# automl/TransformersCanDoBayesianInference

Hardware: NVIDIA H100
Metric: prior-sampled sequences/sec, full training step (prior sample + fwd + bwd + allreduce + clip + Adam) (higher is better)
Workload: dtype bf16

## Files before the change

### transformerscandobayesianinference_b200/csrc/attention_bwd_tc.cu

```cuda
#include "attention_common.cuh"

namespace pfn {

constexpr int AB_ROWS = 64;
constexpr int AB_TILE = AB_ROWS * ATT_ROW_BYTES;
constexpr int AB_THREADS = 3 * 128;
constexpr int AB_DQ_STAGES = 4;
constexpr int AB_DKV_STAGES = 3;
constexpr int AB_DQ_OFF_RING = 4 * AB_TILE;
constexpr int AB_DQ_OFF_BAR = AB_DQ_OFF_RING + AB_DQ_STAGES * 2 * AB_TILE;
constexpr int AB_DQ_SMEM = AB_DQ_OFF_BAR + (2 * AB_DQ_STAGES + 2) * 8 + 1024;
constexpr int AB_DKV_OFF_RING = 4 * AB_TILE;
constexpr int AB_DKV_OFF_STAT = AB_DKV_OFF_RING + AB_DKV_STAGES * 2 * AB_TILE;
constexpr int AB_DKV_OFF_BAR = AB_DKV_OFF_STAT + AB_DKV_STAGES * 2 * AB_ROWS * 4;
constexpr int AB_DKV_SMEM = AB_DKV_OFF_BAR + (2 * AB_DKV_STAGES + 1) * 8 + 1024;
static_assert(AB_DQ_SMEM <= 232448 && AB_DKV_SMEM <= 232448, "the tiles and rings must fit the 227 KB of shared memory");

struct AttnBwdParams {
  int T, B, H, sep;
  float scale, scale_log2;
  const __nv_bfloat16* qkv; int ld_qkv;
  const __nv_bfloat16* dout; int ld_dout;
  __nv_bfloat16* dqkv; int ld_dqkv;
  const float* lse;
  const float* delta;
  int delta_tm;
  float* dq_colsum;
  uint32_t drop_seed; int drop_thr;
  int n_tiles;
  int batch_major;
};

__device__ __forceinline__ float ab_delta(const AttnBwdParams& p, int b, int h, int i) {
  return p.delta_tm ? p.delta[att_tok(i, b, p.T, p.B, 0) * p.H + h] : p.delta[(static_cast<size_t>(b) * p.H + h) * p.T + i];
}

__device__ __forceinline__ uint64_t ab_desc_k(uint32_t tile, int kk) {
  return tc::wgmma_smem_desc(tile + (kk >> 2) * 8192 + (kk & 3) * 32, 16, 1024);
}
__device__ __forceinline__ uint64_t ab_desc_mn(uint32_t tile, int kk) {
  return tc::wgmma_smem_desc(tile + kk * 2048, 8192, 1024);
}
__device__ __forceinline__ uint32_t ab_opaque(uint32_t addr) {
  asm volatile("" : "+r"(addr));
  return addr;
}
__device__ __forceinline__ void ab_mma_n64(float (&d)[32], uint64_t a_desc, uint64_t b_desc, int kk) {
  if (kk == 0) tc::wgmma_m64n64k16<0>(d, a_desc, b_desc);
  else tc::wgmma_m64n64k16<1>(d, a_desc, b_desc);
}

__device__ __forceinline__ void ab_load_tile(uint8_t* dst, const CUtensorMap* m, uint64_t* bar, int col0, int b, int t0) {
  tc::tma_load_3d(dst, m, bar, col0, b, t0);
  tc::tma_load_3d(dst + 8192, m, bar, col0 + 64, b, t0);
}

__global__ void __launch_bounds__(256)
attn_bwd_delta_kernel(const __nv_bfloat16* __restrict__ out, int ld_out, const __nv_bfloat16* __restrict__ dout,
                      int ld_dout, float* __restrict__ delta, int T, int B, int H, int batch_major) {
  const int lane = threadIdx.x & 31;
  const long long warp = (static_cast<long long>(blockIdx.x) * blockDim.x + threadIdx.x) >> 5;
  const long long nwarps = (static_cast<long long>(gridDim.x) * blockDim.x) >> 5;
  const long long rows = static_cast<long long>(T) * B;
  for (long long tok = warp; tok < rows; tok += nwarps) {
    const int t = batch_major ? static_cast<int>(tok % T) : static_cast<int>(tok / B);
    const int b = batch_major ? static_cast<int>(tok / T) : static_cast<int>(tok % B);
    for (int h0 = 0; h0 < H; h0 += 2) {
      const int h = h0 + (lane >> 4);
      float acc = 0.f;
      if (h < H) {
        const int col = h * ATT_DH + (lane & 15) * 8;
        const uint4 pa = *reinterpret_cast<const uint4*>(out + tok * ld_out + col);
        const uint4 pb = *reinterpret_cast<const uint4*>(dout + tok * ld_dout + col);
        const __nv_bfloat162* ha = reinterpret_cast<const __nv_bfloat162*>(&pa);
        const __nv_bfloat162* hb = reinterpret_cast<const __nv_bfloat162*>(&pb);
#pragma unroll
        for (int j = 0; j < 4; ++j) {
          const float2 x = __bfloat1622float2(ha[j]);
          const float2 y = __bfloat1622float2(hb[j]);
          acc = fmaf(x.x, y.x, acc);
          acc = fmaf(x.y, y.y, acc);
        }
      }
#pragma unroll
      for (int o = 8; o > 0; o >>= 1) acc += __shfl_xor_sync(0xffffffffu, acc, o);
      if ((lane & 15) == 0 && h < H) delta[(static_cast<size_t>(b) * H + h) * T + t] = acc;
    }
  }
}

__global__ void __launch_bounds__(AB_THREADS, 1)
attn_bwd_dq_kernel(const __grid_constant__ CUtensorMap tmQ, const __grid_constant__ CUtensorMap tmKV,
                   const __grid_constant__ CUtensorMap tmDO, const AttnBwdParams p) {
  extern __shared__ uint8_t smem_raw[];
  uint8_t* smem = smem_raw + ((1024u - (tc::smem_u32(smem_raw) & 1023u)) & 1023u);
  uint8_t* sQ = smem;
  uint8_t* sD = smem + 2 * AB_TILE;
  uint8_t* sRing = smem + AB_DQ_OFF_RING;
  uint64_t* kv_full = reinterpret_cast<uint64_t*>(smem + AB_DQ_OFF_BAR);
  uint64_t* kv_empty = kv_full + AB_DQ_STAGES;
  uint64_t* q_full = kv_empty + AB_DQ_STAGES;
  uint64_t* q_empty = q_full + 1;
  const int warp = threadIdx.x >> 5, lane = threadIdx.x & 31;
  const int E = p.H * ATT_DH;
  const int nblk = (p.sep + AB_ROWS - 1) / AB_ROWS;
  const int n_units = p.n_tiles * p.B * p.H;
  if (threadIdx.x == 0) {
    for (int s = 0; s < AB_DQ_STAGES; ++s) {
      tc::mbar_init(&kv_full[s], 1);
      tc::mbar_init(&kv_empty[s], 2);
    }
    tc::mbar_init(q_full, 1);
    tc::mbar_init(q_empty, 2);
    tc::mbar_fence_init();
  }
  __syncthreads();

  if (warp >= 8) {
    tc::setmaxnreg_dec<40>();
    if (threadIdx.x == 256) {
      tc::tma_prefetch_desc(&tmQ);
      tc::tma_prefetch_desc(&tmKV);
      tc::tma_prefetch_desc(&tmDO);
      int stage = 0;
      uint32_t phase = 0;
      for (int u = blockIdx.x, it = 0; u < n_units; u += gridDim.x, ++it) {
        const int qt = u % p.n_tiles, bh = u / p.n_tiles;
        const int h = bh % p.H, b = bh / p.H;
        auto load_q = [&]() {
          if (it > 0) tc::mbar_wait_suspend(q_empty, (it - 1) & 1);
          tc::mbar_expect_tx(q_full, 4 * AB_TILE);
          for (int g = 0; g < 2; ++g) {
            ab_load_tile(sQ + g * AB_TILE, &tmQ, q_full, h * ATT_DH, b, qt * 128 + 64 * g);
            ab_load_tile(sD + g * AB_TILE, &tmDO, q_full, h * ATT_DH, b, qt * 128 + 64 * g);
          }
        };
        const int claim_at = min(AB_DQ_STAGES - 1, nblk - 1);
        if (nblk == 0) load_q();
        for (int kb = 0; kb < nblk; ++kb) {
          if (kb == claim_at) load_q();
          tc::mbar_wait_suspend(&kv_empty[stage], phase ^ 1);
          uint8_t* dst = sRing + stage * 2 * AB_TILE;
          tc::mbar_expect_tx(&kv_full[stage], 2 * AB_TILE);
          ab_load_tile(dst, &tmKV, &kv_full[stage], E + h * ATT_DH, b, kb * AB_ROWS);
          ab_load_tile(dst + AB_TILE, &tmKV, &kv_full[stage], 2 * E + h * ATT_DH, b, kb * AB_ROWS);
          if (++stage == AB_DQ_STAGES) { stage = 0; phase ^= 1; }
        }
      }
    }
    return;
  }

  tc::setmaxnreg_inc<232>();
  const int g = warp >> 2, wq = warp & 3;
  const int tid = threadIdx.x & 127;
  const uint32_t q_tile = tc::smem_u32(sQ + g * AB_TILE), d_tile = tc::smem_u32(sD + g * AB_TILE);
  const float dscale = p.drop_thr > 0 ? drop_scale(p.drop_thr) : 1.0f;
  int stage = 0;
  uint32_t phase = 0;
  bool timed_out = false;
  for (int u = blockIdx.x, it = 0; u < n_units && !timed_out; u += gridDim.x, ++it) {
    const int qt = u % p.n_tiles, bh = u / p.n_tiles;
    const int h = bh % p.H, b = bh / p.H;
    const int i0 = qt * 128 + 64 * g + 16 * wq + (lane >> 2);

    float lse2[2], dl[2];
    uint32_t drow[2];
#pragma unroll
    for (int r = 0; r < 2; ++r) {
      const int i = i0 + 8 * r;
      const bool valid = i < p.T;
      lse2[r] = valid ? p.lse[static_cast<size_t>(bh) * p.T + i] * 1.4426950408889634f : INFINITY;
      dl[r] = valid ? ab_delta(p, b, h, i) : 0.f;
      drow[r] = static_cast<uint32_t>(bh) * p.T + i;
    }
    if (!tc::mbar_wait_bounded(q_full, it & 1)) { timed_out = true; break; }

    float dq[64];
    for (int kb = 0; kb < nblk; ++kb) {
      if (!tc::mbar_wait_bounded(&kv_full[stage], phase)) { timed_out = true; break; }
      const uint32_t k_s = tc::smem_u32(sRing + stage * 2 * AB_TILE);
      const uint32_t v_s = k_s + AB_TILE;
      const uint32_t q_s = ab_opaque(q_tile), d_s = ab_opaque(d_tile);
      float s[32], dp[32];
      tc::wgmma_fence();
#pragma unroll
      for (int kk = 0; kk < 8; ++kk) ab_mma_n64(s, ab_desc_k(q_s, kk), ab_desc_k(k_s, kk), kk);
#pragma unroll
      for (int kk = 0; kk < 8; ++kk) ab_mma_n64(dp, ab_desc_k(d_s, kk), ab_desc_k(v_s, kk), kk);
      tc::wgmma_commit();
      tc::wgmma_wait<0>();
      tc::wgmma_fence_regs(s);
      tc::wgmma_fence_regs(dp);
      if (kb == nblk - 1 && tid == 0) tc::mbar_arrive(q_empty);

      uint32_t ads[16];
      const int key0 = kb * AB_ROWS + 2 * (lane & 3);
#pragma unroll
      for (int j = 0; j < 8; ++j)
#pragma unroll
        for (int e = 0; e < 4; e += 2) {
          float v[2];
#pragma unroll
          for (int c = 0; c < 2; ++c) {
            const int key = key0 + 8 * j + c;
            const float pr = key < p.sep ? fast_ex2(fmaf(s[4 * j + e + c], p.scale_log2, -lse2[e >> 1])) : 0.f;
            const float mk = p.drop_thr > 0 ? (drop_keep(p.drop_seed, drow[e >> 1], key, p.drop_thr) ? dscale : 0.f) : 1.f;
            v[c] = pr * fmaf(mk, dp[4 * j + e + c], -dl[e >> 1]) * p.scale;
          }
          ads[2 * j + (e >> 1)] = tc::pack_bf16x2(v[0], v[1]);
        }
      tc::wgmma_fence();
#pragma unroll
      for (int kk = 0; kk < 4; ++kk) tc::wgmma_m64n128k16_rs(dq, ads + 4 * kk, ab_desc_mn(k_s, kk), kb > 0 || kk > 0);
      tc::wgmma_commit();
      tc::wgmma_wait<0>();
      if (tid == 0) tc::mbar_arrive(&kv_empty[stage]);
      if (++stage == AB_DQ_STAGES) { stage = 0; phase ^= 1; }
    }
    tc::wgmma_fence_regs(dq);
    if (nblk == 0 && tid == 0) tc::mbar_arrive(q_empty);

    float cs[16][2];
#pragma unroll
    for (int j = 0; j < 16; ++j) cs[j][0] = cs[j][1] = 0.f;
#pragma unroll
    for (int r = 0; r < 2; ++r) {
      const int i = i0 + 8 * r;
      const bool valid = i < p.T;
      const bool diag = valid && i >= p.sep;
      const size_t tok = att_tok(valid ? i : 0, b, p.T, p.B, p.batch_major);
      const __nv_bfloat16* qrow = p.qkv + tok * p.ld_qkv + h * ATT_DH;
      const __nv_bfloat16* drw = p.dout + tok * p.ld_dout + h * ATT_DH;
      __nv_bfloat16* grow = p.dqkv + tok * p.ld_dqkv + h * ATT_DH;
      float sd = 0.f, dpd = 0.f;
      if (diag) {
#pragma unroll
        for (int j = 0; j < 16; ++j) {
          const float2 q = att_ld2(qrow, j, lane), k = att_ld2(qrow + E, j, lane);
          const float2 gr = att_ld2(drw, j, lane), v = att_ld2(qrow + 2 * E, j, lane);
          sd = fmaf(q.x, k.x, fmaf(q.y, k.y, sd));
          dpd = fmaf(gr.x, v.x, fmaf(gr.y, v.y, dpd));
        }
      }
      sd = quad_sum(sd);
      dpd = quad_sum(dpd);
      float ds = 0.f;
      if (diag) {
        const float pr = fast_ex2(fmaf(sd, p.scale_log2, -lse2[r]));
        const float mk = p.drop_thr > 0 ? (drop_keep(p.drop_seed, drow[r], i, p.drop_thr) ? dscale : 0.f) : 1.f;
        ds = pr * fmaf(mk, dpd, -dl[r]) * p.scale;
        const float pm = pr * mk;
#pragma unroll
        for (int j = 0; j < 16; ++j) {
          const float2 q = att_ld2(qrow, j, lane), gr = att_ld2(drw, j, lane);
          att_st2(grow + E, j, lane, ds * q.x, ds * q.y);
          att_st2(grow + 2 * E, j, lane, pm * gr.x, pm * gr.y);
        }
      }
      if (valid) {
#pragma unroll
        for (int j = 0; j < 16; ++j) {
          float x = nblk > 0 ? dq[4 * j + 2 * r] : 0.f, y = nblk > 0 ? dq[4 * j + 2 * r + 1] : 0.f;
          if (diag) {
            const float2 k = att_ld2(qrow + E, j, lane);
            x = fmaf(ds, k.x, x);
            y = fmaf(ds, k.y, y);
          }
          att_st2(grow, j, lane, x, y);
          cs[j][0] += __bfloat162float(__float2bfloat16_rn(x));
          cs[j][1] += __bfloat162float(__float2bfloat16_rn(y));
        }
      }
    }
    if (p.dq_colsum != nullptr) {
#pragma unroll
      for (int j = 0; j < 16; ++j)
#pragma unroll
        for (int e = 0; e < 2; ++e) {
          float v = cs[j][e];
          v += __shfl_xor_sync(0xffffffffu, v, 4);
          v += __shfl_xor_sync(0xffffffffu, v, 8);
          v += __shfl_xor_sync(0xffffffffu, v, 16);
          if (lane < 4) atomicAdd(p.dq_colsum + h * ATT_DH + 8 * j + 2 * lane + e, v);
        }
    }
  }
  if (timed_out) asm volatile("trap;");
}

__global__ void __launch_bounds__(AB_THREADS, 1)
attn_bwd_dkv_kernel(const __grid_constant__ CUtensorMap tmQ, const __grid_constant__ CUtensorMap tmKV,
                    const __grid_constant__ CUtensorMap tmDO, const AttnBwdParams p) {
  extern __shared__ uint8_t smem_raw[];
  uint8_t* smem = smem_raw + ((1024u - (tc::smem_u32(smem_raw) & 1023u)) & 1023u);
  uint8_t* sK = smem;
  uint8_t* sV = smem + 2 * AB_TILE;
  uint8_t* sRing = smem + AB_DKV_OFF_RING;
  float* sStat = reinterpret_cast<float*>(smem + AB_DKV_OFF_STAT);
  uint64_t* full = reinterpret_cast<uint64_t*>(smem + AB_DKV_OFF_BAR);
  uint64_t* empty = full + AB_DKV_STAGES;
  uint64_t* kv_bar = empty + AB_DKV_STAGES;
  const int warp = threadIdx.x >> 5, lane = threadIdx.x & 31;
  const int kt = static_cast<int>(blockIdx.x) % p.n_tiles;
  const int bh = static_cast<int>(blockIdx.x) / p.n_tiles;
  const int h = bh % p.H, b = bh / p.H;
  const int E = p.H * ATT_DH;
  const int nqb = (p.T + AB_ROWS - 1) / AB_ROWS;
  if (threadIdx.x == 0) {
    for (int s = 0; s < AB_DKV_STAGES; ++s) {
      tc::mbar_init(&full[s], 1 + AB_ROWS);
      tc::mbar_init(&empty[s], 2);
    }
    tc::mbar_init(kv_bar, 1);
    tc::mbar_fence_init();
  }
  __syncthreads();

  if (warp >= 8) {
    tc::setmaxnreg_dec<40>();
    const int pt = threadIdx.x - 256;
    int stage = 0;
    uint32_t phase = 0;
    if (pt == 0) {
      tc::tma_prefetch_desc(&tmQ);
      tc::tma_prefetch_desc(&tmKV);
      tc::tma_prefetch_desc(&tmDO);
      tc::mbar_expect_tx(kv_bar, 4 * AB_TILE);
      for (int g = 0; g < 2; ++g) {
        const int j0 = kt * 128 + 64 * g;
        ab_load_tile(sK + g * AB_TILE, &tmKV, kv_bar, E + h * ATT_DH, b, j0);
        ab_load_tile(sV + g * AB_TILE, &tmKV, kv_bar, 2 * E + h * ATT_DH, b, j0);
      }
      for (int qb = 0; qb < nqb; ++qb) {
        tc::mbar_wait_suspend(&empty[stage], phase ^ 1);
        uint8_t* dst = sRing + stage * 2 * AB_TILE;
        tc::mbar_expect_tx(&full[stage], 2 * AB_TILE);
        ab_load_tile(dst, &tmQ, &full[stage], h * ATT_DH, b, qb * AB_ROWS);
        ab_load_tile(dst + AB_TILE, &tmDO, &full[stage], h * ATT_DH, b, qb * AB_ROWS);
        if (++stage == AB_DKV_STAGES) { stage = 0; phase ^= 1; }
      }
    } else if (pt >= 64) {
      const int r = pt - 64;
      for (int qb = 0; qb < nqb; ++qb) {
        const int i = qb * AB_ROWS + r;
        const bool valid = i < p.T;
        const float l2 = valid ? p.lse[static_cast<size_t>(bh) * p.T + i] * 1.4426950408889634f : INFINITY;
        const float dl = valid ? ab_delta(p, b, h, i) : 0.f;
        tc::mbar_wait_suspend(&empty[stage], phase ^ 1);
        sStat[stage * 2 * AB_ROWS + r] = l2;
        sStat[stage * 2 * AB_ROWS + AB_ROWS + r] = dl;
        tc::mbar_arrive(&full[stage]);
        if (++stage == AB_DKV_STAGES) { stage = 0; phase ^= 1; }
      }
    }
    return;
  }

  tc::setmaxnreg_inc<232>();
  const int g = warp >> 2, wq = warp & 3;
  const int tid = threadIdx.x & 127;
  const uint32_t k_tile = tc::smem_u32(sK + g * AB_TILE), v_tile = tc::smem_u32(sV + g * AB_TILE);
  const float dscale = p.drop_thr > 0 ? drop_scale(p.drop_thr) : 1.0f;
  const int key_a = kt * 128 + 64 * g + 16 * wq + (lane >> 2);
  const uint32_t drow_base = static_cast<uint32_t>(bh) * p.T;
  tc::mbar_wait(kv_bar, 0);

  float dk[64], dv[64];
  int stage = 0;
  uint32_t phase = 0;
  bool timed_out = false;
  for (int qb = 0; qb < nqb; ++qb) {
    if (!tc::mbar_wait_bounded(&full[stage], phase)) { timed_out = true; break; }
    const uint32_t q_s = tc::smem_u32(sRing + stage * 2 * AB_TILE);
    const uint32_t d_s = q_s + AB_TILE;
    const uint32_t k_s = ab_opaque(k_tile), v_s = ab_opaque(v_tile);
    const float* st_lse = sStat + stage * 2 * AB_ROWS;
    const float* st_dl = st_lse + AB_ROWS;
    float s[32], dp[32];
    tc::wgmma_fence();
#pragma unroll
    for (int kk = 0; kk < 8; ++kk) ab_mma_n64(s, ab_desc_k(k_s, kk), ab_desc_k(q_s, kk), kk);
#pragma unroll
    for (int kk = 0; kk < 8; ++kk) ab_mma_n64(dp, ab_desc_k(v_s, kk), ab_desc_k(d_s, kk), kk);
    tc::wgmma_commit();
    tc::wgmma_wait<0>();
    tc::wgmma_fence_regs(s);
    tc::wgmma_fence_regs(dp);

#pragma unroll
    for (int kk = 0; kk < 4; ++kk) {
      uint32_t ap[4], as[4];
#pragma unroll
      for (int jj = 0; jj < 2; ++jj)
#pragma unroll
        for (int e = 0; e < 4; e += 2) {
          const int j = 2 * kk + jj;
          float pm[2], ds[2];
#pragma unroll
          for (int c = 0; c < 2; ++c) {
            const int ci = 8 * j + 2 * (lane & 3) + c;
            const int i = qb * AB_ROWS + ci;
            const float pr = fast_ex2(fmaf(s[4 * j + e + c], p.scale_log2, -st_lse[ci]));
            const float mk = p.drop_thr > 0 ? (drop_keep(p.drop_seed, drow_base + i, key_a + 8 * (e >> 1), p.drop_thr) ? dscale : 0.f) : 1.f;
            ds[c] = pr * fmaf(mk, dp[4 * j + e + c], -st_dl[ci]) * p.scale;
            pm[c] = pr * mk;
          }
          ap[2 * jj + (e >> 1)] = tc::pack_bf16x2(pm[0], pm[1]);
          as[2 * jj + (e >> 1)] = tc::pack_bf16x2(ds[0], ds[1]);
        }
      tc::wgmma_fence();
      tc::wgmma_m64n128k16_rs(dv, ap, ab_desc_mn(d_s, kk), qb > 0 || kk > 0);
      tc::wgmma_m64n128k16_rs(dk, as, ab_desc_mn(q_s, kk), qb > 0 || kk > 0);
    }
    tc::wgmma_commit();
    tc::wgmma_wait<0>();
    if (tid == 0) tc::mbar_arrive(&empty[stage]);
    if (++stage == AB_DKV_STAGES) { stage = 0; phase ^= 1; }
  }
  tc::wgmma_fence_regs(dk);
  tc::wgmma_fence_regs(dv);

#pragma unroll
  for (int r = 0; r < 2; ++r) {
    const int key = key_a + 8 * r;
    if (key < p.sep) {
      __nv_bfloat16* grow = p.dqkv + att_tok(key, b, p.T, p.B, p.batch_major) * p.ld_dqkv + h * ATT_DH;
#pragma unroll
      for (int j = 0; j < 16; ++j) {
        att_st2(grow + E, j, lane, dk[4 * j + 2 * r], dk[4 * j + 2 * r + 1]);
        att_st2(grow + 2 * E, j, lane, dv[4 * j + 2 * r], dv[4 * j + 2 * r + 1]);
      }
    }
  }
  if (timed_out) asm volatile("trap;");
}

static int ab_tensor_map(CUtensorMap* m, const void* base, int cols, int ld, int T, int B, int t_extent, int batch_major) {
  const uint64_t row = static_cast<uint64_t>(ld) * 2;
  const uint64_t dims[3] = {static_cast<uint64_t>(cols), static_cast<uint64_t>(B), static_cast<uint64_t>(t_extent)};
  const uint64_t strides[3] = {0, batch_major ? row * T : row, batch_major ? row : row * B};
  const uint32_t box[3] = {64, 1, AB_ROWS};
  return make_tensor_map(m, base, false, 3, dims, strides, box, true);
}

}

using namespace pfn;

extern "C" int pfn_attention_bwd_tc(const pfn_attn_desc* d, void* stream) {
  if (int rc = check_tc_attn(d, true, "attention_bwd_tc")) return rc;
  PFN_CHECK_ARG(!(d->delta_token_major && d->batch_major), "attention_bwd_tc: a token-major delta implies the reference token order");
  AttnBwdParams p;
  p.T = d->T; p.B = d->B; p.H = d->H; p.sep = d->sep;
  p.scale = d->scale; p.scale_log2 = d->scale * 1.4426950408889634f;
  p.qkv = reinterpret_cast<const __nv_bfloat16*>(d->qkv); p.ld_qkv = d->ld_qkv;
  p.dout = reinterpret_cast<const __nv_bfloat16*>(d->dout); p.ld_dout = d->ld_dout;
  p.dqkv = reinterpret_cast<__nv_bfloat16*>(d->dqkv); p.ld_dqkv = d->ld_dqkv;
  p.lse = d->lse; p.delta = d->delta; p.dq_colsum = d->dq_colsum; p.delta_tm = d->delta_token_major;
  p.drop_seed = d->drop_seed; p.drop_thr = d->drop_thr;
  p.batch_major = d->batch_major;
  const int E = d->H * ATT_DH;
  CUtensorMap tmQ, tmKV, tmDO;
  if (int rc = ab_tensor_map(&tmQ, d->qkv, 3 * E, d->ld_qkv, d->T, d->B, d->T, d->batch_major)) return rc;
  if (int rc = ab_tensor_map(&tmKV, d->qkv, 3 * E, d->ld_qkv, d->T, d->B, d->sep > 0 ? d->sep : 1, d->batch_major)) return rc;
  if (int rc = ab_tensor_map(&tmDO, d->dout, E, d->ld_dout, d->T, d->B, d->T, d->batch_major)) return rc;
  static bool attr_set[64] = {};
  if (first_use_on_device(attr_set)) {
    PFN_CUDA_OK(cudaFuncSetAttribute(attn_bwd_dq_kernel, cudaFuncAttributeMaxDynamicSharedMemorySize, AB_DQ_SMEM));
    PFN_CUDA_OK(cudaFuncSetAttribute(attn_bwd_dkv_kernel, cudaFuncAttributeMaxDynamicSharedMemorySize, AB_DKV_SMEM));
  }
  cudaStream_t s = reinterpret_cast<cudaStream_t>(stream);
  if (!d->delta_token_major) {
    const long long rows = static_cast<long long>(d->T) * d->B;
    long long grid = (rows + 7) / 8;
    if (grid > 8LL * num_sms()) grid = 8LL * num_sms();
    attn_bwd_delta_kernel<<<static_cast<int>(grid), 256, 0, s>>>(reinterpret_cast<const __nv_bfloat16*>(d->out), d->ld_out,
                                                                 p.dout, p.ld_dout, d->delta, d->T, d->B, d->H, d->batch_major);
    PFN_LAUNCH_OK();
  }
  p.n_tiles = (d->T + 127) / 128;
  const long long units = static_cast<long long>(p.n_tiles) * d->B * d->H;
  PFN_CHECK_ARG(units < (1LL << 31), "attention_bwd_tc: too many tiles");
  const int grid_dq = units < num_sms() ? static_cast<int>(units) : num_sms();
  attn_bwd_dq_kernel<<<static_cast<unsigned>(grid_dq), AB_THREADS, AB_DQ_SMEM, s>>>(tmQ, tmKV, tmDO, p);
  PFN_LAUNCH_OK();
  if (d->sep > 0) {
    p.n_tiles = (d->sep + 127) / 128;
    const long long grid = static_cast<long long>(p.n_tiles) * d->B * d->H;
    attn_bwd_dkv_kernel<<<static_cast<unsigned>(grid), AB_THREADS, AB_DKV_SMEM, s>>>(tmQ, tmKV, tmDO, p);
    PFN_LAUNCH_OK();
  }
  return 0;
}
```

### transformerscandobayesianinference_b200/csrc/attention_common.cuh

```cuda
#pragma once
#include "common.cuh"
#include "dropout.cuh"
#include "tc_common.cuh"
#include "../../include/pfn_b200.h"

namespace pfn {

constexpr int ATT_DH = 128;
constexpr int ATT_ROW_BYTES = ATT_DH * 2;

int check_attn_desc_public(const pfn_attn_desc* d, bool bwd, const char* who);

__device__ __forceinline__ uint32_t att_sw(int r, int c) {
  return static_cast<uint32_t>(r * ATT_ROW_BYTES + ((((c >> 3) ^ (r & 7))) << 4) + (c & 7) * 2);
}

__device__ __forceinline__ size_t att_tok(int t, int b, int T, int B, int batch_major) {
  return batch_major ? static_cast<size_t>(b) * T + t : static_cast<size_t>(t) * B + b;
}

template <int NROWS>
__device__ __forceinline__ void att_load_tile(uint8_t* tile, const __nv_bfloat16* base, int ld, int col0, int t0, int t_end,
                                              int b, int T, int B, int batch_major) {
  const uint32_t s = tc::smem_u32(tile);
#pragma unroll
  for (int k = 0; k < NROWS * 16 / 128; ++k) {
    const int idx = static_cast<int>(threadIdx.x) + 128 * k;
    const int r = idx >> 4, c = idx & 15;
    const int t = t0 + r;
    const bool ok = t < t_end;
    const __nv_bfloat16* src = ok ? base + att_tok(t, b, T, B, batch_major) * ld + col0 + c * 8 : base;
    tc::cp_async16(s + att_sw(r, c * 8), src, ok ? 16u : 0u);
  }
}

__device__ __forceinline__ void att_frag_a(uint32_t (&a)[4], uint32_t tile, int r0, int c0, int lane) {
  tc::ldmatrix_x4(a, tile + att_sw(r0 + (lane & 15), c0 + ((lane >> 4) << 3)));
}
__device__ __forceinline__ void att_frag_b(uint32_t (&b)[4], uint32_t tile, int n0, int k0, int lane) {
  tc::ldmatrix_x4(b, tile + att_sw(n0 + (lane & 7) + ((lane >> 4) << 3), k0 + (((lane >> 3) & 1) << 3)));
}
__device__ __forceinline__ void att_frag_bt(uint32_t (&b)[4], uint32_t tile, int k0, int n0, int lane) {
  tc::ldmatrix_x4_trans(b, tile + att_sw(k0 + (lane & 7) + (((lane >> 3) & 1) << 3), n0 + ((lane >> 4) << 3)));
}

__device__ __forceinline__ float2 att_ld2(const __nv_bfloat16* row, int j, int lane) {
  return __bfloat1622float2(*reinterpret_cast<const __nv_bfloat162*>(row + 8 * j + 2 * (lane & 3)));
}
__device__ __forceinline__ void att_st2(__nv_bfloat16* row, int j, int lane, float x, float y) {
  *reinterpret_cast<uint32_t*>(row + 8 * j + 2 * (lane & 3)) = tc::pack_bf16x2(x, y);
}
__device__ __forceinline__ float quad_sum(float v) {
  v += __shfl_xor_sync(0xffffffffu, v, 1);
  return v + __shfl_xor_sync(0xffffffffu, v, 2);
}
__device__ __forceinline__ float quad_max(float v) {
  v = fmaxf(v, __shfl_xor_sync(0xffffffffu, v, 1));
  return fmaxf(v, __shfl_xor_sync(0xffffffffu, v, 2));
}

static inline int check_tc_attn(const pfn_attn_desc* d, bool bwd, const char* who) {
  if (int rc = check_attn_desc_public(d, bwd, who)) return rc;
  PFN_CHECK_ARG(d->dtype == PFN_BF16, "%s: bf16 only", who);
  PFN_CHECK_ARG(d->dh == ATT_DH, "%s: head dim %d unsupported (built for 128)", who, d->dh);
  PFN_CHECK_ARG(d->ld_qkv % 8 == 0 && d->ld_out % 8 == 0, "%s: leading dims must be multiples of 8", who);
  PFN_CHECK_ARG(((reinterpret_cast<uintptr_t>(d->qkv) | reinterpret_cast<uintptr_t>(d->out)) & 15) == 0,
                "%s: qkv/out must be 16-byte aligned", who);
  if (bwd) {
    PFN_CHECK_ARG(d->ld_dout % 8 == 0 && d->ld_dqkv % 8 == 0, "%s: leading dims must be multiples of 8", who);
    PFN_CHECK_ARG(((reinterpret_cast<uintptr_t>(d->dout) | reinterpret_cast<uintptr_t>(d->dqkv)) & 15) == 0,
                  "%s: dout/dqkv must be 16-byte aligned", who);
  }
  return 0;
}

}
```

### transformerscandobayesianinference_b200/csrc/attention_tc.cu

```cuda
#include "attention_common.cuh"

namespace pfn {

constexpr int ATT_BM = 64;
constexpr int ATT_BN = 64;
constexpr int ATT_TILE_BYTES = ATT_BM * ATT_ROW_BYTES;
constexpr int ATT_FWD_SMEM = 5 * ATT_TILE_BYTES;

struct AttnFwdParams {
  int T, B, H, sep;
  float scale_log2;
  const __nv_bfloat16* qkv; int ld_qkv;
  __nv_bfloat16* out; int ld_out;
  float* lse;
  int n_qtiles;
  int batch_major;
  uint32_t drop_seed; int drop_thr;
};

__global__ void __launch_bounds__(128, 2)
attn_fwd_tc_kernel(const AttnFwdParams p) {
  extern __shared__ __align__(128) uint8_t smem[];
  uint8_t* sQ = smem;
  uint8_t* sK = smem + ATT_TILE_BYTES;
  uint8_t* sV = smem + 3 * ATT_TILE_BYTES;
  const int warp = threadIdx.x >> 5, lane = threadIdx.x & 31;
  const int qt = static_cast<int>(blockIdx.x) % p.n_qtiles;
  const int bh = static_cast<int>(blockIdx.x) / p.n_qtiles;
  const int h = bh % p.H, b = bh / p.H;
  const int E = p.H * ATT_DH;
  const int i0 = qt * ATT_BM;
  const int nblk = (p.sep + ATT_BN - 1) / ATT_BN;

  att_load_tile<ATT_BM>(sQ, p.qkv, p.ld_qkv, h * ATT_DH, i0, p.T, b, p.T, p.B, p.batch_major);
  if (nblk > 0) {
    att_load_tile<ATT_BN>(sK, p.qkv, p.ld_qkv, E + h * ATT_DH, 0, p.sep, b, p.T, p.B, p.batch_major);
    att_load_tile<ATT_BN>(sV, p.qkv, p.ld_qkv, 2 * E + h * ATT_DH, 0, p.sep, b, p.T, p.B, p.batch_major);
  }
  tc::cp_async_commit();

  float o[16][4];
#pragma unroll
  for (int j = 0; j < 16; ++j) o[j][0] = o[j][1] = o[j][2] = o[j][3] = 0.f;
  float m[2] = {-INFINITY, -INFINITY}, l[2] = {0.f, 0.f};
  const int r0 = 16 * warp;
  const uint32_t drow0 = static_cast<uint32_t>(bh) * p.T + i0 + r0 + (lane >> 2);
  const uint32_t q_s = tc::smem_u32(sQ);

  for (int kb = 0; kb < nblk; ++kb) {
    if (kb + 1 < nblk) {
      const int nb = (kb + 1) & 1;
      att_load_tile<ATT_BN>(sK + nb * ATT_TILE_BYTES, p.qkv, p.ld_qkv, E + h * ATT_DH, (kb + 1) * ATT_BN, p.sep, b, p.T, p.B, p.batch_major);
      att_load_tile<ATT_BN>(sV + nb * ATT_TILE_BYTES, p.qkv, p.ld_qkv, 2 * E + h * ATT_DH, (kb + 1) * ATT_BN, p.sep, b, p.T, p.B, p.batch_major);
      tc::cp_async_commit();
      tc::cp_async_wait<1>();
    } else {
      tc::cp_async_wait<0>();
    }
    __syncthreads();
    const uint32_t k_s = tc::smem_u32(sK + (kb & 1) * ATT_TILE_BYTES);
    const uint32_t v_s = tc::smem_u32(sV + (kb & 1) * ATT_TILE_BYTES);

    float s[8][4];
#pragma unroll
    for (int j = 0; j < 8; ++j) s[j][0] = s[j][1] = s[j][2] = s[j][3] = 0.f;
#pragma unroll
    for (int kk = 0; kk < 8; ++kk) {
      uint32_t a[4];
      att_frag_a(a, q_s, r0, kk * 16, lane);
#pragma unroll
      for (int np = 0; np < 4; ++np) {
        uint32_t bb[4];
        att_frag_b(bb, k_s, np * 16, kk * 16, lane);
        tc::mma_bf16_16816(s[2 * np], a, bb[0], bb[1]);
        tc::mma_bf16_16816(s[2 * np + 1], a, bb[2], bb[3]);
      }
    }
    const int key0 = kb * ATT_BN + 2 * (lane & 3);
    float mx[2] = {-INFINITY, -INFINITY};
#pragma unroll
    for (int j = 0; j < 8; ++j)
#pragma unroll
      for (int e = 0; e < 4; ++e) {
        const bool ok = key0 + 8 * j + (e & 1) < p.sep;
        s[j][e] = ok ? s[j][e] * p.scale_log2 : -INFINITY;
        mx[e >> 1] = fmaxf(mx[e >> 1], s[j][e]);
      }
    float corr[2];
#pragma unroll
    for (int r = 0; r < 2; ++r) {
      const float mn = fmaxf(m[r], quad_max(mx[r]));
      corr[r] = fast_ex2(m[r] - mn);
      m[r] = mn;
      l[r] *= corr[r];
    }
#pragma unroll
    for (int j = 0; j < 8; ++j)
#pragma unroll
      for (int e = 0; e < 4; ++e) {
        const float pr = fast_ex2(s[j][e] - m[e >> 1]);
        l[e >> 1] += pr;
        if (p.drop_thr > 0 && !drop_keep(p.drop_seed, drow0 + 8 * (e >> 1), key0 + 8 * j + (e & 1), p.drop_thr)) s[j][e] = 0.f;
        else s[j][e] = pr;
      }
#pragma unroll
    for (int j = 0; j < 16; ++j) {
      o[j][0] *= corr[0]; o[j][1] *= corr[0];
      o[j][2] *= corr[1]; o[j][3] *= corr[1];
    }
#pragma unroll
    for (int kk = 0; kk < 4; ++kk) {
      uint32_t a[4];
      a[0] = tc::pack_bf16x2(s[2 * kk][0], s[2 * kk][1]);
      a[1] = tc::pack_bf16x2(s[2 * kk][2], s[2 * kk][3]);
      a[2] = tc::pack_bf16x2(s[2 * kk + 1][0], s[2 * kk + 1][1]);
      a[3] = tc::pack_bf16x2(s[2 * kk + 1][2], s[2 * kk + 1][3]);
#pragma unroll
      for (int dp = 0; dp < 8; ++dp) {
        uint32_t bb[4];
        att_frag_bt(bb, v_s, kk * 16, dp * 16, lane);
        tc::mma_bf16_16816(o[2 * dp], a, bb[0], bb[1]);
        tc::mma_bf16_16816(o[2 * dp + 1], a, bb[2], bb[3]);
      }
    }
    __syncthreads();
  }

  const float dscale = p.drop_thr > 0 ? drop_scale(p.drop_thr) : 1.0f;
#pragma unroll
  for (int r = 0; r < 2; ++r) {
    const int i = i0 + r0 + (lane >> 2) + 8 * r;
    float lr = quad_sum(l[r]);
    const bool valid = i < p.T;
    const bool diag = valid && i >= p.sep;
    const __nv_bfloat16* qrow = p.qkv + att_tok(valid ? i : 0, b, p.T, p.B, p.batch_major) * p.ld_qkv + h * ATT_DH;
    float sd = 0.f;
    if (diag) {
#pragma unroll
      for (int j = 0; j < 16; ++j) {
        const float2 q = att_ld2(qrow, j, lane), k = att_ld2(qrow + E, j, lane);
        sd = fmaf(q.x, k.x, fmaf(q.y, k.y, sd));
      }
    }
    sd = quad_sum(sd) * p.scale_log2;
    if (diag) {
      const float mn = fmaxf(m[r], sd);
      const float c = fast_ex2(m[r] - mn);
      const float pr = fast_ex2(sd - mn);
      lr = lr * c + pr;
      m[r] = mn;
      const float pd = (p.drop_thr > 0 && !drop_keep(p.drop_seed, drow0 + 8 * r, i, p.drop_thr)) ? 0.f : pr;
#pragma unroll
      for (int j = 0; j < 16; ++j) {
        const float2 v = att_ld2(qrow + 2 * E, j, lane);
        o[j][2 * r] = fmaf(pd, v.x, o[j][2 * r] * c);
        o[j][2 * r + 1] = fmaf(pd, v.y, o[j][2 * r + 1] * c);
      }
    }
    if (valid) {
      const float inv = dscale / lr;
      __nv_bfloat16* orow = p.out + att_tok(i, b, p.T, p.B, p.batch_major) * p.ld_out + h * ATT_DH;
#pragma unroll
      for (int j = 0; j < 16; ++j) att_st2(orow, j, lane, o[j][2 * r] * inv, o[j][2 * r + 1] * inv);
      if ((lane & 3) == 0) p.lse[static_cast<size_t>(bh) * p.T + i] = (m[r] + __log2f(lr)) * 0.69314718055994531f;
    }
  }
}

}

using namespace pfn;

extern "C" int pfn_attention_fwd_tc(const pfn_attn_desc* d, void* stream) {
  if (int rc = check_tc_attn(d, false, "attention_fwd_tc")) return rc;
  AttnFwdParams p;
  p.T = d->T; p.B = d->B; p.H = d->H; p.sep = d->sep;
  p.scale_log2 = d->scale * 1.4426950408889634f;
  p.qkv = reinterpret_cast<const __nv_bfloat16*>(d->qkv); p.ld_qkv = d->ld_qkv;
  p.out = reinterpret_cast<__nv_bfloat16*>(d->out); p.ld_out = d->ld_out;
  p.lse = d->lse;
  p.n_qtiles = (d->T + ATT_BM - 1) / ATT_BM;
  p.batch_major = d->batch_major;
  p.drop_seed = d->drop_seed; p.drop_thr = d->drop_thr;
  const long long grid = static_cast<long long>(p.n_qtiles) * d->B * d->H;
  PFN_CHECK_ARG(grid < (1LL << 31), "attention_fwd_tc: too many tiles");
  static bool attr_set[64] = {};
  if (first_use_on_device(attr_set)) {
    PFN_CUDA_OK(cudaFuncSetAttribute(attn_fwd_tc_kernel, cudaFuncAttributeMaxDynamicSharedMemorySize, ATT_FWD_SMEM));
  }
  attn_fwd_tc_kernel<<<static_cast<unsigned>(grid), 128, ATT_FWD_SMEM, reinterpret_cast<cudaStream_t>(stream)>>>(p);
  PFN_LAUNCH_OK();
  return 0;
}
```

### transformerscandobayesianinference_b200/csrc/tc_common.cuh

```cuda
#pragma once
#include <cuda.h>
#include <cuda_bf16.h>
#include <cuda_runtime.h>
#include <stdint.h>

namespace pfn {
namespace tc {

__device__ __forceinline__ uint32_t smem_u32(const void* p) {
  return static_cast<uint32_t>(__cvta_generic_to_shared(p));
}

__device__ __forceinline__ void mbar_init(uint64_t* bar, uint32_t count) {
  asm volatile("mbarrier.init.shared::cta.b64 [%0], %1;" ::"r"(smem_u32(bar)), "r"(count) : "memory");
}
__device__ __forceinline__ void mbar_fence_init() {
  asm volatile("fence.mbarrier_init.release.cluster;" ::: "memory");
}
__device__ __forceinline__ void mbar_expect_tx(uint64_t* bar, uint32_t bytes) {
  asm volatile("mbarrier.arrive.expect_tx.shared::cta.b64 _, [%0], %1;" ::"r"(smem_u32(bar)), "r"(bytes) : "memory");
}
__device__ __forceinline__ void mbar_arrive(uint64_t* bar) {
  asm volatile("mbarrier.arrive.shared::cta.b64 _, [%0];" ::"r"(smem_u32(bar)) : "memory");
}
__device__ __forceinline__ bool mbar_try_wait(uint64_t* bar, uint32_t parity) {
  uint32_t ok;
  asm volatile(
      "{\n\t.reg .pred P;\n\t"
      "mbarrier.test_wait.parity.shared::cta.b64 P, [%1], %2;\n\t"
      "selp.u32 %0, 1, 0, P;\n\t}"
      : "=r"(ok)
      : "r"(smem_u32(bar)), "r"(parity)
      : "memory");
  return ok != 0;
}
#ifndef PFN_MBAR_SPIN_LIMIT
#define PFN_MBAR_SPIN_LIMIT (1u << 28)
#endif
__device__ __forceinline__ void mbar_wait(uint64_t* bar, uint32_t parity) {
  uint32_t spins = 0;
  while (!mbar_try_wait(bar, parity)) {
    if (++spins > PFN_MBAR_SPIN_LIMIT) asm volatile("trap;");
  }
}
__device__ __forceinline__ bool mbar_wait_bounded(uint64_t* bar, uint32_t parity) {
  uint32_t spins = 0;
  while (!mbar_try_wait(bar, parity)) {
    if (++spins > PFN_MBAR_SPIN_LIMIT) return false;
  }
  return true;
}

__device__ __forceinline__ void mbar_wait_suspend(uint64_t* bar, uint32_t parity) {
  uint32_t ok = 0, spins = 0;
  while (true) {
    asm volatile(
        "{\n\t.reg .pred P;\n\t"
        "mbarrier.try_wait.parity.shared::cta.b64 P, [%1], %2;\n\t"
        "selp.u32 %0, 1, 0, P;\n\t}"
        : "=r"(ok)
        : "r"(smem_u32(bar)), "r"(parity)
        : "memory");
    if (ok) break;
    if (++spins > PFN_MBAR_SPIN_LIMIT) asm volatile("trap;");
  }
}
__device__ __forceinline__ void tma_prefetch_desc(const CUtensorMap* m) {
  asm volatile("prefetch.tensormap [%0];" ::"l"(reinterpret_cast<uint64_t>(m)) : "memory");
}
__device__ __forceinline__ void tma_load_2d(void* smem_dst, const CUtensorMap* m, uint64_t* bar, int c0, int c1) {
  asm volatile(
      "cp.async.bulk.tensor.2d.shared::cluster.global.tile.mbarrier::complete_tx::bytes [%0], [%1, {%3, %4}], [%2];"
      ::"r"(smem_u32(smem_dst)), "l"(reinterpret_cast<uint64_t>(m)), "r"(smem_u32(bar)), "r"(c0), "r"(c1)
      : "memory");
}
__device__ __forceinline__ void tma_load_3d(void* smem_dst, const CUtensorMap* m, uint64_t* bar, int c0, int c1, int c2) {
  asm volatile(
      "cp.async.bulk.tensor.3d.shared::cluster.global.tile.mbarrier::complete_tx::bytes [%0], [%1, {%3, %4, %5}], [%2];"
      ::"r"(smem_u32(smem_dst)), "l"(reinterpret_cast<uint64_t>(m)), "r"(smem_u32(bar)), "r"(c0), "r"(c1), "r"(c2)
      : "memory");
}
__device__ __forceinline__ void tma_store_2d(const CUtensorMap* m, const void* smem_src, int c0, int c1) {
  asm volatile("cp.async.bulk.tensor.2d.global.shared::cta.tile.bulk_group [%0, {%2, %3}], [%1];"
               ::"l"(reinterpret_cast<uint64_t>(m)), "r"(smem_u32(smem_src)), "r"(c0), "r"(c1)
               : "memory");
}
__device__ __forceinline__ void tma_reduce_add_2d(const CUtensorMap* m, const void* smem_src, int c0, int c1) {
  asm volatile("cp.reduce.async.bulk.tensor.2d.global.shared::cta.add.tile.bulk_group [%0, {%2, %3}], [%1];"
               ::"l"(reinterpret_cast<uint64_t>(m)), "r"(smem_u32(smem_src)), "r"(c0), "r"(c1)
               : "memory");
}
__device__ __forceinline__ void bulk_commit() { asm volatile("cp.async.bulk.commit_group;" ::: "memory"); }
template <int N>
__device__ __forceinline__ void bulk_wait_read() {
  asm volatile("cp.async.bulk.wait_group.read %0;" ::"n"(N) : "memory");
}
template <int N>
__device__ __forceinline__ void bulk_wait() {
  asm volatile("cp.async.bulk.wait_group %0;" ::"n"(N) : "memory");
}
__device__ __forceinline__ void fence_proxy_async_smem() { asm volatile("fence.proxy.async.shared::cta;" ::: "memory"); }

__device__ __forceinline__ void named_bar_sync(int id, int threads) {
  asm volatile("bar.sync %0, %1;" ::"r"(id), "r"(threads) : "memory");
}
__device__ __forceinline__ void named_bar_arrive(int id, int threads) {
  asm volatile("bar.arrive %0, %1;" ::"r"(id), "r"(threads) : "memory");
}
template <int N>
__device__ __forceinline__ void setmaxnreg_dec() { asm volatile("setmaxnreg.dec.sync.aligned.u32 %0;" ::"n"(N)); }
template <int N>
__device__ __forceinline__ void setmaxnreg_inc() { asm volatile("setmaxnreg.inc.sync.aligned.u32 %0;" ::"n"(N)); }

__device__ __forceinline__ uint32_t pack_bf16x2(float lo, float hi) {
  __nv_bfloat162 t = __floats2bfloat162_rn(lo, hi);
  return *reinterpret_cast<uint32_t*>(&t);
}

__device__ __forceinline__ uint64_t wgmma_smem_desc(uint32_t smem_addr, uint32_t lbo_bytes, uint32_t sbo_bytes) {
  return (1ull << 62) | (static_cast<uint64_t>((sbo_bytes >> 4) & 0x3FFF) << 32) |
         (static_cast<uint64_t>((lbo_bytes >> 4) & 0x3FFF) << 16) | static_cast<uint64_t>((smem_addr >> 4) & 0x3FFF);
}

__device__ __forceinline__ void wgmma_fence() { asm volatile("wgmma.fence.sync.aligned;" ::: "memory"); }
__device__ __forceinline__ void wgmma_commit() { asm volatile("wgmma.commit_group.sync.aligned;" ::: "memory"); }
template <int N>
__device__ __forceinline__ void wgmma_wait() {
  asm volatile("wgmma.wait_group.sync.aligned %0;" ::"n"(N) : "memory");
}
template <int N>
__device__ __forceinline__ void wgmma_fence_regs(float (&d)[N]) {
#pragma unroll
  for (int i = 0; i < N; ++i) asm volatile("" : "+f"(d[i])::"memory");
}

template <int TA, int TB>
__device__ __forceinline__ void wgmma_m64n128k16(float (&d)[64], uint64_t a_desc, uint64_t b_desc, uint32_t accumulate) {
  asm volatile(
      "{\n\t.reg .pred p;\n\t"
      "setp.ne.b32 p, %66, 0;\n\t"
      "wgmma.mma_async.sync.aligned.m64n128k16.f32.bf16.bf16 "
      "{%0, %1, %2, %3, %4, %5, %6, %7, %8, %9, %10, %11, %12, %13, %14, %15, "
      "%16, %17, %18, %19, %20, %21, %22, %23, %24, %25, %26, %27, %28, %29, %30, %31, "
      "%32, %33, %34, %35, %36, %37, %38, %39, %40, %41, %42, %43, %44, %45, %46, %47, "
      "%48, %49, %50, %51, %52, %53, %54, %55, %56, %57, %58, %59, %60, %61, %62, %63}, "
      "%64, %65, p, 1, 1, %67, %68;\n\t}"
      : "+f"(d[0]), "+f"(d[1]), "+f"(d[2]), "+f"(d[3]), "+f"(d[4]), "+f"(d[5]), "+f"(d[6]), "+f"(d[7]),
        "+f"(d[8]), "+f"(d[9]), "+f"(d[10]), "+f"(d[11]), "+f"(d[12]), "+f"(d[13]), "+f"(d[14]), "+f"(d[15]),
        "+f"(d[16]), "+f"(d[17]), "+f"(d[18]), "+f"(d[19]), "+f"(d[20]), "+f"(d[21]), "+f"(d[22]), "+f"(d[23]),
        "+f"(d[24]), "+f"(d[25]), "+f"(d[26]), "+f"(d[27]), "+f"(d[28]), "+f"(d[29]), "+f"(d[30]), "+f"(d[31]),
        "+f"(d[32]), "+f"(d[33]), "+f"(d[34]), "+f"(d[35]), "+f"(d[36]), "+f"(d[37]), "+f"(d[38]), "+f"(d[39]),
        "+f"(d[40]), "+f"(d[41]), "+f"(d[42]), "+f"(d[43]), "+f"(d[44]), "+f"(d[45]), "+f"(d[46]), "+f"(d[47]),
        "+f"(d[48]), "+f"(d[49]), "+f"(d[50]), "+f"(d[51]), "+f"(d[52]), "+f"(d[53]), "+f"(d[54]), "+f"(d[55]),
        "+f"(d[56]), "+f"(d[57]), "+f"(d[58]), "+f"(d[59]), "+f"(d[60]), "+f"(d[61]), "+f"(d[62]), "+f"(d[63])
      : "l"(a_desc), "l"(b_desc), "r"(accumulate), "n"(TA), "n"(TB));
}

#define PFN_WGMMA_D32(C)                                                                                          \
  C(d[0]), C(d[1]), C(d[2]), C(d[3]), C(d[4]), C(d[5]), C(d[6]), C(d[7]), C(d[8]), C(d[9]), C(d[10]), C(d[11]),   \
      C(d[12]), C(d[13]), C(d[14]), C(d[15]), C(d[16]), C(d[17]), C(d[18]), C(d[19]), C(d[20]), C(d[21]),         \
      C(d[22]), C(d[23]), C(d[24]), C(d[25]), C(d[26]), C(d[27]), C(d[28]), C(d[29]), C(d[30]), C(d[31])
#define PFN_WGMMA_M64N64K16(SCALE_D)                                                                              \
  "wgmma.mma_async.sync.aligned.m64n64k16.f32.bf16.bf16 "                                                         \
  "{%0, %1, %2, %3, %4, %5, %6, %7, %8, %9, %10, %11, %12, %13, %14, %15, "                                       \
  "%16, %17, %18, %19, %20, %21, %22, %23, %24, %25, %26, %27, %28, %29, %30, %31}, %32, %33, " SCALE_D ", 1, 1, 0, 0;"
template <int ACCUMULATE>
__device__ __forceinline__ void wgmma_m64n64k16(float (&d)[32], uint64_t a_desc, uint64_t b_desc) {
  if constexpr (ACCUMULATE) {
    asm volatile(PFN_WGMMA_M64N64K16("1") : PFN_WGMMA_D32("+f") : "l"(a_desc), "l"(b_desc));
  } else {
    asm volatile(PFN_WGMMA_M64N64K16("0") : PFN_WGMMA_D32("=f") : "l"(a_desc), "l"(b_desc));
  }
}
#undef PFN_WGMMA_M64N64K16
#undef PFN_WGMMA_D32

__device__ __forceinline__ void wgmma_m64n128k16_rs(float (&d)[64], const uint32_t* a, uint64_t b_desc, uint32_t accumulate) {
  asm volatile(
      "{\n\t.reg .pred p;\n\t"
      "setp.ne.b32 p, %69, 0;\n\t"
      "wgmma.mma_async.sync.aligned.m64n128k16.f32.bf16.bf16 "
      "{%0, %1, %2, %3, %4, %5, %6, %7, %8, %9, %10, %11, %12, %13, %14, %15, "
      "%16, %17, %18, %19, %20, %21, %22, %23, %24, %25, %26, %27, %28, %29, %30, %31, "
      "%32, %33, %34, %35, %36, %37, %38, %39, %40, %41, %42, %43, %44, %45, %46, %47, "
      "%48, %49, %50, %51, %52, %53, %54, %55, %56, %57, %58, %59, %60, %61, %62, %63}, "
      "{%64, %65, %66, %67}, %68, p, 1, 1, 1;\n\t}"
      : "+f"(d[0]), "+f"(d[1]), "+f"(d[2]), "+f"(d[3]), "+f"(d[4]), "+f"(d[5]), "+f"(d[6]), "+f"(d[7]),
        "+f"(d[8]), "+f"(d[9]), "+f"(d[10]), "+f"(d[11]), "+f"(d[12]), "+f"(d[13]), "+f"(d[14]), "+f"(d[15]),
        "+f"(d[16]), "+f"(d[17]), "+f"(d[18]), "+f"(d[19]), "+f"(d[20]), "+f"(d[21]), "+f"(d[22]), "+f"(d[23]),
        "+f"(d[24]), "+f"(d[25]), "+f"(d[26]), "+f"(d[27]), "+f"(d[28]), "+f"(d[29]), "+f"(d[30]), "+f"(d[31]),
        "+f"(d[32]), "+f"(d[33]), "+f"(d[34]), "+f"(d[35]), "+f"(d[36]), "+f"(d[37]), "+f"(d[38]), "+f"(d[39]),
        "+f"(d[40]), "+f"(d[41]), "+f"(d[42]), "+f"(d[43]), "+f"(d[44]), "+f"(d[45]), "+f"(d[46]), "+f"(d[47]),
        "+f"(d[48]), "+f"(d[49]), "+f"(d[50]), "+f"(d[51]), "+f"(d[52]), "+f"(d[53]), "+f"(d[54]), "+f"(d[55]),
        "+f"(d[56]), "+f"(d[57]), "+f"(d[58]), "+f"(d[59]), "+f"(d[60]), "+f"(d[61]), "+f"(d[62]), "+f"(d[63])
      : "r"(a[0]), "r"(a[1]), "r"(a[2]), "r"(a[3]), "l"(b_desc), "r"(accumulate));
}

__device__ __forceinline__ void mma_bf16_16816(float (&c)[4], const uint32_t (&a)[4], uint32_t b0, uint32_t b1) {
  asm volatile(
      "mma.sync.aligned.m16n8k16.row.col.f32.bf16.bf16.f32 {%0, %1, %2, %3}, {%4, %5, %6, %7}, {%8, %9}, "
      "{%0, %1, %2, %3};"
      : "+f"(c[0]), "+f"(c[1]), "+f"(c[2]), "+f"(c[3])
      : "r"(a[0]), "r"(a[1]), "r"(a[2]), "r"(a[3]), "r"(b0), "r"(b1));
}
__device__ __forceinline__ void ldmatrix_x4(uint32_t (&r)[4], uint32_t addr) {
  asm volatile("ldmatrix.sync.aligned.m8n8.x4.shared.b16 {%0, %1, %2, %3}, [%4];"
               : "=r"(r[0]), "=r"(r[1]), "=r"(r[2]), "=r"(r[3])
               : "r"(addr));
}
__device__ __forceinline__ void ldmatrix_x4_trans(uint32_t (&r)[4], uint32_t addr) {
  asm volatile("ldmatrix.sync.aligned.m8n8.x4.trans.shared.b16 {%0, %1, %2, %3}, [%4];"
               : "=r"(r[0]), "=r"(r[1]), "=r"(r[2]), "=r"(r[3])
               : "r"(addr));
}
__device__ __forceinline__ void cp_async16(uint32_t dst, const void* src, uint32_t src_bytes) {
  asm volatile("cp.async.cg.shared.global [%0], [%1], 16, %2;" ::"r"(dst), "l"(src), "r"(src_bytes) : "memory");
}
__device__ __forceinline__ void cp_async_commit() { asm volatile("cp.async.commit_group;" ::: "memory"); }
template <int N>
__device__ __forceinline__ void cp_async_wait() {
  asm volatile("cp.async.wait_group %0;" ::"n"(N) : "memory");
}

}

int make_tensor_map(CUtensorMap* out, const void* base, bool f32, int rank, const uint64_t* dims,
                    const uint64_t* strides_bytes, const uint32_t* box, bool swizzle128);

}
```

Measured before the change: 2286.

## Rewrite attention forward as persistent warp-specialized WGMMA kernel with TMA pipeline

Replaces the mma.sync/ldmatrix attention forward kernel, which used cp.async double buffering and one 64-row tile per block, with a persistent kernel. A TMA producer warp feeds a 4-stage K/V ring and two consumer warpgroups compute QK^T and PV with wgmma, with output staged in shared memory and written back through a TMA store. Descriptor, tile-load and tensor-map helpers move from the backward file into a shared header. The aim is higher tensor-core throughput and less load overhead in the forward pass, at the cost of more complex mbarrier synchronization and one block per SM.

```diff
diff --git a/transformerscandobayesianinference_b200/csrc/attention_bwd_tc.cu b/transformerscandobayesianinference_b200/csrc/attention_bwd_tc.cu
--- a/transformerscandobayesianinference_b200/csrc/attention_bwd_tc.cu
+++ b/transformerscandobayesianinference_b200/csrc/attention_bwd_tc.cu
@@ -2,8 +2,8 @@
 
 namespace pfn {
 
-constexpr int AB_ROWS = 64;
-constexpr int AB_TILE = AB_ROWS * ATT_ROW_BYTES;
+constexpr int AB_ROWS = ATT_TILE_ROWS;
+constexpr int AB_TILE = ATT_TILE;
 constexpr int AB_THREADS = 3 * 128;
 constexpr int AB_DQ_STAGES = 4;
 constexpr int AB_DKV_STAGES = 3;
@@ -33,26 +33,6 @@
 
 __device__ __forceinline__ float ab_delta(const AttnBwdParams& p, int b, int h, int i) {
   return p.delta_tm ? p.delta[att_tok(i, b, p.T, p.B, 0) * p.H + h] : p.delta[(static_cast<size_t>(b) * p.H + h) * p.T + i];
-}
-
-__device__ __forceinline__ uint64_t ab_desc_k(uint32_t tile, int kk) {
-  return tc::wgmma_smem_desc(tile + (kk >> 2) * 8192 + (kk & 3) * 32, 16, 1024);
-}
-__device__ __forceinline__ uint64_t ab_desc_mn(uint32_t tile, int kk) {
-  return tc::wgmma_smem_desc(tile + kk * 2048, 8192, 1024);
-}
-__device__ __forceinline__ uint32_t ab_opaque(uint32_t addr) {
-  asm volatile("" : "+r"(addr));
-  return addr;
-}
-__device__ __forceinline__ void ab_mma_n64(float (&d)[32], uint64_t a_desc, uint64_t b_desc, int kk) {
-  if (kk == 0) tc::wgmma_m64n64k16<0>(d, a_desc, b_desc);
-  else tc::wgmma_m64n64k16<1>(d, a_desc, b_desc);
-}
-
-__device__ __forceinline__ void ab_load_tile(uint8_t* dst, const CUtensorMap* m, uint64_t* bar, int col0, int b, int t0) {
-  tc::tma_load_3d(dst, m, bar, col0, b, t0);
-  tc::tma_load_3d(dst + 8192, m, bar, col0 + 64, b, t0);
 }
 
 __global__ void __launch_bounds__(256)
@@ -131,8 +111,8 @@
           if (it > 0) tc::mbar_wait_suspend(q_empty, (it - 1) & 1);
           tc::mbar_expect_tx(q_full, 4 * AB_TILE);
           for (int g = 0; g < 2; ++g) {
-            ab_load_tile(sQ + g * AB_TILE, &tmQ, q_full, h * ATT_DH, b, qt * 128 + 64 * g);
-            ab_load_tile(sD + g * AB_TILE, &tmDO, q_full, h * ATT_DH, b, qt * 128 + 64 * g);
+            att_load_tile(sQ + g * AB_TILE, &tmQ, q_full, h * ATT_DH, b, qt * 128 + 64 * g);
+            att_load_tile(sD + g * AB_TILE, &tmDO, q_full, h * ATT_DH, b, qt * 128 + 64 * g);
           }
         };
         const int claim_at = min(AB_DQ_STAGES - 1, nblk - 1);
@@ -142,8 +122,8 @@
           tc::mbar_wait_suspend(&kv_empty[stage], phase ^ 1);
           uint8_t* dst = sRing + stage * 2 * AB_TILE;
           tc::mbar_expect_tx(&kv_full[stage], 2 * AB_TILE);
-          ab_load_tile(dst, &tmKV, &kv_full[stage], E + h * ATT_DH, b, kb * AB_ROWS);
-          ab_load_tile(dst + AB_TILE, &tmKV, &kv_full[stage], 2 * E + h * ATT_DH, b, kb * AB_ROWS);
+          att_load_tile(dst, &tmKV, &kv_full[stage], E + h * ATT_DH, b, kb * AB_ROWS);
+          att_load_tile(dst + AB_TILE, &tmKV, &kv_full[stage], 2 * E + h * ATT_DH, b, kb * AB_ROWS);
           if (++stage == AB_DQ_STAGES) { stage = 0; phase ^= 1; }
         }
       }
@@ -181,13 +161,13 @@
       if (!tc::mbar_wait_bounded(&kv_full[stage], phase)) { timed_out = true; break; }
       const uint32_t k_s = tc::smem_u32(sRing + stage * 2 * AB_TILE);
       const uint32_t v_s = k_s + AB_TILE;
-      const uint32_t q_s = ab_opaque(q_tile), d_s = ab_opaque(d_tile);
+      const uint32_t q_s = att_opaque(q_tile), d_s = att_opaque(d_tile);
       float s[32], dp[32];
       tc::wgmma_fence();
 #pragma unroll
-      for (int kk = 0; kk < 8; ++kk) ab_mma_n64(s, ab_desc_k(q_s, kk), ab_desc_k(k_s, kk), kk);
-#pragma unroll
-      for (int kk = 0; kk < 8; ++kk) ab_mma_n64(dp, ab_desc_k(d_s, kk), ab_desc_k(v_s, kk), kk);
+      for (int kk = 0; kk < 8; ++kk) att_mma_n64(s, att_desc_k(q_s, kk), att_desc_k(k_s, kk), kk);
+#pragma unroll
+      for (int kk = 0; kk < 8; ++kk) att_mma_n64(dp, att_desc_k(d_s, kk), att_desc_k(v_s, kk), kk);
       tc::wgmma_commit();
       tc::wgmma_wait<0>();
       tc::wgmma_fence_regs(s);
@@ -212,7 +192,7 @@
         }
       tc::wgmma_fence();
 #pragma unroll
-      for (int kk = 0; kk < 4; ++kk) tc::wgmma_m64n128k16_rs(dq, ads + 4 * kk, ab_desc_mn(k_s, kk), kb > 0 || kk > 0);
+      for (int kk = 0; kk < 4; ++kk) tc::wgmma_m64n128k16_rs(dq, ads + 4 * kk, att_desc_mn(k_s, kk), kb > 0 || kk > 0);
       tc::wgmma_commit();
       tc::wgmma_wait<0>();
       if (tid == 0) tc::mbar_arrive(&kv_empty[stage]);
@@ -329,15 +309,15 @@
       tc::mbar_expect_tx(kv_bar, 4 * AB_TILE);
       for (int g = 0; g < 2; ++g) {
         const int j0 = kt * 128 + 64 * g;
-        ab_load_tile(sK + g * AB_TILE, &tmKV, kv_bar, E + h * ATT_DH, b, j0);
-        ab_load_tile(sV + g * AB_TILE, &tmKV, kv_bar, 2 * E + h * ATT_DH, b, j0);
+        att_load_tile(sK + g * AB_TILE, &tmKV, kv_bar, E + h * ATT_DH, b, j0);
+        att_load_tile(sV + g * AB_TILE, &tmKV, kv_bar, 2 * E + h * ATT_DH, b, j0);
       }
       for (int qb = 0; qb < nqb; ++qb) {
         tc::mbar_wait_suspend(&empty[stage], phase ^ 1);
         uint8_t* dst = sRing + stage * 2 * AB_TILE;
         tc::mbar_expect_tx(&full[stage], 2 * AB_TILE);
-        ab_load_tile(dst, &tmQ, &full[stage], h * ATT_DH, b, qb * AB_ROWS);
-        ab_load_tile(dst + AB_TILE, &tmDO, &full[stage], h * ATT_DH, b, qb * AB_ROWS);
+        att_load_tile(dst, &tmQ, &full[stage], h * ATT_DH, b, qb * AB_ROWS);
+        att_load_tile(dst + AB_TILE, &tmDO, &full[stage], h * ATT_DH, b, qb * AB_ROWS);
         if (++stage == AB_DKV_STAGES) { stage = 0; phase ^= 1; }
       }
     } else if (pt >= 64) {
@@ -374,15 +354,15 @@
     if (!tc::mbar_wait_bounded(&full[stage], phase)) { timed_out = true; break; }
     const uint32_t q_s = tc::smem_u32(sRing + stage * 2 * AB_TILE);
     const uint32_t d_s = q_s + AB_TILE;
-    const uint32_t k_s = ab_opaque(k_tile), v_s = ab_opaque(v_tile);
+    const uint32_t k_s = att_opaque(k_tile), v_s = att_opaque(v_tile);
     const float* st_lse = sStat + stage * 2 * AB_ROWS;
     const float* st_dl = st_lse + AB_ROWS;
     float s[32], dp[32];
     tc::wgmma_fence();
 #pragma unroll
-    for (int kk = 0; kk < 8; ++kk) ab_mma_n64(s, ab_desc_k(k_s, kk), ab_desc_k(q_s, kk), kk);
-#pragma unroll
-    for (int kk = 0; kk < 8; ++kk) ab_mma_n64(dp, ab_desc_k(v_s, kk), ab_desc_k(d_s, kk), kk);
+    for (int kk = 0; kk < 8; ++kk) att_mma_n64(s, att_desc_k(k_s, kk), att_desc_k(q_s, kk), kk);
+#pragma unroll
+    for (int kk = 0; kk < 8; ++kk) att_mma_n64(dp, att_desc_k(v_s, kk), att_desc_k(d_s, kk), kk);
     tc::wgmma_commit();
     tc::wgmma_wait<0>();
     tc::wgmma_fence_regs(s);
@@ -410,8 +390,8 @@
           as[2 * jj + (e >> 1)] = tc::pack_bf16x2(ds[0], ds[1]);
         }
       tc::wgmma_fence();
-      tc::wgmma_m64n128k16_rs(dv, ap, ab_desc_mn(d_s, kk), qb > 0 || kk > 0);
-      tc::wgmma_m64n128k16_rs(dk, as, ab_desc_mn(q_s, kk), qb > 0 || kk > 0);
+      tc::wgmma_m64n128k16_rs(dv, ap, att_desc_mn(d_s, kk), qb > 0 || kk > 0);
+      tc::wgmma_m64n128k16_rs(dk, as, att_desc_mn(q_s, kk), qb > 0 || kk > 0);
     }
     tc::wgmma_commit();
     tc::wgmma_wait<0>();
@@ -434,14 +414,6 @@
     }
   }
   if (timed_out) asm volatile("trap;");
-}
-
-static int ab_tensor_map(CUtensorMap* m, const void* base, int cols, int ld, int T, int B, int t_extent, int batch_major) {
-  const uint64_t row = static_cast<uint64_t>(ld) * 2;
-  const uint64_t dims[3] = {static_cast<uint64_t>(cols), static_cast<uint64_t>(B), static_cast<uint64_t>(t_extent)};
-  const uint64_t strides[3] = {0, batch_major ? row * T : row, batch_major ? row : row * B};
-  const uint32_t box[3] = {64, 1, AB_ROWS};
-  return make_tensor_map(m, base, false, 3, dims, strides, box, true);
 }
 
 }
@@ -462,9 +434,8 @@
   p.batch_major = d->batch_major;
   const int E = d->H * ATT_DH;
   CUtensorMap tmQ, tmKV, tmDO;
-  if (int rc = ab_tensor_map(&tmQ, d->qkv, 3 * E, d->ld_qkv, d->T, d->B, d->T, d->batch_major)) return rc;
-  if (int rc = ab_tensor_map(&tmKV, d->qkv, 3 * E, d->ld_qkv, d->T, d->B, d->sep > 0 ? d->sep : 1, d->batch_major)) return rc;
-  if (int rc = ab_tensor_map(&tmDO, d->dout, E, d->ld_dout, d->T, d->B, d->T, d->batch_major)) return rc;
+  if (int rc = att_qkv_maps(d, &tmQ, &tmKV)) return rc;
+  if (int rc = att_tensor_map(&tmDO, d->dout, E, d->ld_dout, d->T, d->B, d->T, d->batch_major)) return rc;
   static bool attr_set[64] = {};
   if (first_use_on_device(attr_set)) {
     PFN_CUDA_OK(cudaFuncSetAttribute(attn_bwd_dq_kernel, cudaFuncAttributeMaxDynamicSharedMemorySize, AB_DQ_SMEM));
diff --git a/transformerscandobayesianinference_b200/csrc/attention_common.cuh b/transformerscandobayesianinference_b200/csrc/attention_common.cuh
--- a/transformerscandobayesianinference_b200/csrc/attention_common.cuh
+++ b/transformerscandobayesianinference_b200/csrc/attention_common.cuh
@@ -8,40 +8,33 @@
 
 constexpr int ATT_DH = 128;
 constexpr int ATT_ROW_BYTES = ATT_DH * 2;
+constexpr int ATT_TILE_ROWS = 64;
+constexpr int ATT_TILE = ATT_TILE_ROWS * ATT_ROW_BYTES;
 
 int check_attn_desc_public(const pfn_attn_desc* d, bool bwd, const char* who);
-
-__device__ __forceinline__ uint32_t att_sw(int r, int c) {
-  return static_cast<uint32_t>(r * ATT_ROW_BYTES + ((((c >> 3) ^ (r & 7))) << 4) + (c & 7) * 2);
-}
 
 __device__ __forceinline__ size_t att_tok(int t, int b, int T, int B, int batch_major) {
   return batch_major ? static_cast<size_t>(b) * T + t : static_cast<size_t>(t) * B + b;
 }
 
-template <int NROWS>
-__device__ __forceinline__ void att_load_tile(uint8_t* tile, const __nv_bfloat16* base, int ld, int col0, int t0, int t_end,
-                                              int b, int T, int B, int batch_major) {
-  const uint32_t s = tc::smem_u32(tile);
-#pragma unroll
-  for (int k = 0; k < NROWS * 16 / 128; ++k) {
-    const int idx = static_cast<int>(threadIdx.x) + 128 * k;
-    const int r = idx >> 4, c = idx & 15;
-    const int t = t0 + r;
-    const bool ok = t < t_end;
-    const __nv_bfloat16* src = ok ? base + att_tok(t, b, T, B, batch_major) * ld + col0 + c * 8 : base;
-    tc::cp_async16(s + att_sw(r, c * 8), src, ok ? 16u : 0u);
-  }
+__device__ __forceinline__ uint64_t att_desc_k(uint32_t tile, int kk) {
+  return tc::wgmma_smem_desc(tile + (kk >> 2) * 8192 + (kk & 3) * 32, 16, 1024);
+}
+__device__ __forceinline__ uint64_t att_desc_mn(uint32_t tile, int kk) {
+  return tc::wgmma_smem_desc(tile + kk * 2048, 8192, 1024);
+}
+__device__ __forceinline__ uint32_t att_opaque(uint32_t addr) {
+  asm volatile("" : "+r"(addr));
+  return addr;
+}
+__device__ __forceinline__ void att_mma_n64(float (&d)[32], uint64_t a_desc, uint64_t b_desc, int kk) {
+  if (kk == 0) tc::wgmma_m64n64k16<0>(d, a_desc, b_desc);
+  else tc::wgmma_m64n64k16<1>(d, a_desc, b_desc);
 }
 
-__device__ __forceinline__ void att_frag_a(uint32_t (&a)[4], uint32_t tile, int r0, int c0, int lane) {
-  tc::ldmatrix_x4(a, tile + att_sw(r0 + (lane & 15), c0 + ((lane >> 4) << 3)));
-}
-__device__ __forceinline__ void att_frag_b(uint32_t (&b)[4], uint32_t tile, int n0, int k0, int lane) {
-  tc::ldmatrix_x4(b, tile + att_sw(n0 + (lane & 7) + ((lane >> 4) << 3), k0 + (((lane >> 3) & 1) << 3)));
-}
-__device__ __forceinline__ void att_frag_bt(uint32_t (&b)[4], uint32_t tile, int k0, int n0, int lane) {
-  tc::ldmatrix_x4_trans(b, tile + att_sw(k0 + (lane & 7) + (((lane >> 3) & 1) << 3), n0 + ((lane >> 4) << 3)));
+__device__ __forceinline__ void att_load_tile(uint8_t* dst, const CUtensorMap* m, uint64_t* bar, int col0, int b, int t0) {
+  tc::tma_load_3d(dst, m, bar, col0, b, t0);
+  tc::tma_load_3d(dst + 8192, m, bar, col0 + 64, b, t0);
 }
 
 __device__ __forceinline__ float2 att_ld2(const __nv_bfloat16* row, int j, int lane) {
@@ -74,4 +67,19 @@
   return 0;
 }
 
+static inline int att_tensor_map(CUtensorMap* m, const void* base, int cols, int ld, int T, int B, int t_extent,
+                                 int batch_major) {
+  const uint64_t row = static_cast<uint64_t>(ld) * 2;
+  const uint64_t dims[3] = {static_cast<uint64_t>(cols), static_cast<uint64_t>(B), static_cast<uint64_t>(t_extent)};
+  const uint64_t strides[3] = {0, batch_major ? row * T : row, batch_major ? row : row * B};
+  const uint32_t box[3] = {64, 1, ATT_TILE_ROWS};
+  return make_tensor_map(m, base, false, 3, dims, strides, box, true);
 }
+
+static inline int att_qkv_maps(const pfn_attn_desc* d, CUtensorMap* tmQ, CUtensorMap* tmKV) {
+  const int E = d->H * ATT_DH;
+  if (int rc = att_tensor_map(tmQ, d->qkv, 3 * E, d->ld_qkv, d->T, d->B, d->T, d->batch_major)) return rc;
+  return att_tensor_map(tmKV, d->qkv, 3 * E, d->ld_qkv, d->T, d->B, d->sep > 0 ? d->sep : 1, d->batch_major);
+}
+
+}
diff --git a/transformerscandobayesianinference_b200/csrc/attention_tc.cu b/transformerscandobayesianinference_b200/csrc/attention_tc.cu
--- a/transformerscandobayesianinference_b200/csrc/attention_tc.cu
+++ b/transformerscandobayesianinference_b200/csrc/attention_tc.cu
@@ -2,169 +2,234 @@
 
 namespace pfn {
 
-constexpr int ATT_BM = 64;
-constexpr int ATT_BN = 64;
-constexpr int ATT_TILE_BYTES = ATT_BM * ATT_ROW_BYTES;
-constexpr int ATT_FWD_SMEM = 5 * ATT_TILE_BYTES;
+constexpr int AF_THREADS = 3 * 128;
+constexpr int AF_STAGES = 4;
+constexpr int AF_OFF_STG = 2 * ATT_TILE;
+constexpr int AF_OFF_RING = 4 * ATT_TILE;
+constexpr int AF_OFF_BAR = AF_OFF_RING + AF_STAGES * 2 * ATT_TILE;
+constexpr int AF_SMEM = AF_OFF_BAR + (2 * AF_STAGES + 2) * 8 + 1024;
+static_assert(AF_SMEM <= 232448, "the tiles and the ring must fit the 227 KB of shared memory");
 
 struct AttnFwdParams {
   int T, B, H, sep;
   float scale_log2;
   const __nv_bfloat16* qkv; int ld_qkv;
-  __nv_bfloat16* out; int ld_out;
   float* lse;
-  int n_qtiles;
+  int n_tiles;
   int batch_major;
   uint32_t drop_seed; int drop_thr;
 };
 
-__global__ void __launch_bounds__(128, 2)
-attn_fwd_tc_kernel(const AttnFwdParams p) {
-  extern __shared__ __align__(128) uint8_t smem[];
+__global__ void __launch_bounds__(AF_THREADS, 1)
+attn_fwd_kernel(const __grid_constant__ CUtensorMap tmQ, const __grid_constant__ CUtensorMap tmKV,
+                const __grid_constant__ CUtensorMap tmO, const AttnFwdParams p) {
+  extern __shared__ uint8_t smem_raw[];
+  uint8_t* smem = smem_raw + ((1024u - (tc::smem_u32(smem_raw) & 1023u)) & 1023u);
   uint8_t* sQ = smem;
-  uint8_t* sK = smem + ATT_TILE_BYTES;
-  uint8_t* sV = smem + 3 * ATT_TILE_BYTES;
+  uint8_t* sStg = smem + AF_OFF_STG;
+  uint8_t* sRing = smem + AF_OFF_RING;
+  uint64_t* kv_full = reinterpret_cast<uint64_t*>(smem + AF_OFF_BAR);
+  uint64_t* kv_empty = kv_full + AF_STAGES;
+  uint64_t* q_full = kv_empty + AF_STAGES;
+  uint64_t* q_empty = q_full + 1;
   const int warp = threadIdx.x >> 5, lane = threadIdx.x & 31;
-  const int qt = static_cast<int>(blockIdx.x) % p.n_qtiles;
-  const int bh = static_cast<int>(blockIdx.x) / p.n_qtiles;
-  const int h = bh % p.H, b = bh / p.H;
   const int E = p.H * ATT_DH;
-  const int i0 = qt * ATT_BM;
-  const int nblk = (p.sep + ATT_BN - 1) / ATT_BN;
-
-  att_load_tile<ATT_BM>(sQ, p.qkv, p.ld_qkv, h * ATT_DH, i0, p.T, b, p.T, p.B, p.batch_major);
-  if (nblk > 0) {
-    att_load_tile<ATT_BN>(sK, p.qkv, p.ld_qkv, E + h * ATT_DH, 0, p.sep, b, p.T, p.B, p.batch_major);
-    att_load_tile<ATT_BN>(sV, p.qkv, p.ld_qkv, 2 * E + h * ATT_DH, 0, p.sep, b, p.T, p.B, p.batch_major);
-  }
-  tc::cp_async_commit();
-
-  float o[16][4];
-#pragma unroll
-  for (int j = 0; j < 16; ++j) o[j][0] = o[j][1] = o[j][2] = o[j][3] = 0.f;
-  float m[2] = {-INFINITY, -INFINITY}, l[2] = {0.f, 0.f};
-  const int r0 = 16 * warp;
-  const uint32_t drow0 = static_cast<uint32_t>(bh) * p.T + i0 + r0 + (lane >> 2);
-  const uint32_t q_s = tc::smem_u32(sQ);
-
-  for (int kb = 0; kb < nblk; ++kb) {
-    if (kb + 1 < nblk) {
-      const int nb = (kb + 1) & 1;
-      att_load_tile<ATT_BN>(sK + nb * ATT_TILE_BYTES, p.qkv, p.ld_qkv, E + h * ATT_DH, (kb + 1) * ATT_BN, p.sep, b, p.T, p.B, p.batch_major);
-      att_load_tile<ATT_BN>(sV + nb * ATT_TILE_BYTES, p.qkv, p.ld_qkv, 2 * E + h * ATT_DH, (kb + 1) * ATT_BN, p.sep, b, p.T, p.B, p.batch_major);
-      tc::cp_async_commit();
-      tc::cp_async_wait<1>();
-    } else {
-      tc::cp_async_wait<0>();
-    }
-    __syncthreads();
-    const uint32_t k_s = tc::smem_u32(sK + (kb & 1) * ATT_TILE_BYTES);
-    const uint32_t v_s = tc::smem_u32(sV + (kb & 1) * ATT_TILE_BYTES);
-
-    float s[8][4];
-#pragma unroll
-    for (int j = 0; j < 8; ++j) s[j][0] = s[j][1] = s[j][2] = s[j][3] = 0.f;
-#pragma unroll
-    for (int kk = 0; kk < 8; ++kk) {
-      uint32_t a[4];
-      att_frag_a(a, q_s, r0, kk * 16, lane);
-#pragma unroll
-      for (int np = 0; np < 4; ++np) {
-        uint32_t bb[4];
-        att_frag_b(bb, k_s, np * 16, kk * 16, lane);
-        tc::mma_bf16_16816(s[2 * np], a, bb[0], bb[1]);
-        tc::mma_bf16_16816(s[2 * np + 1], a, bb[2], bb[3]);
-      }
-    }
-    const int key0 = kb * ATT_BN + 2 * (lane & 3);
-    float mx[2] = {-INFINITY, -INFINITY};
-#pragma unroll
-    for (int j = 0; j < 8; ++j)
-#pragma unroll
-      for (int e = 0; e < 4; ++e) {
-        const bool ok = key0 + 8 * j + (e & 1) < p.sep;
-        s[j][e] = ok ? s[j][e] * p.scale_log2 : -INFINITY;
-        mx[e >> 1] = fmaxf(mx[e >> 1], s[j][e]);
-      }
+  const int nblk = (p.sep + ATT_TILE_ROWS - 1) / ATT_TILE_ROWS;
+  const int n_units = p.n_tiles * p.B * p.H;
+  if (threadIdx.x == 0) {
+    for (int s = 0; s < AF_STAGES; ++s) {
+      tc::mbar_init(&kv_full[s], 1);
+      tc::mbar_init(&kv_empty[s], 2);
+    }
+    tc::mbar_init(q_full, 1);
+    tc::mbar_init(q_empty, 2);
+    tc::mbar_fence_init();
+  }
+  __syncthreads();
+
+  if (warp >= 8) {
+    tc::setmaxnreg_dec<40>();
+    if (threadIdx.x == 256) {
+      tc::tma_prefetch_desc(&tmQ);
+      tc::tma_prefetch_desc(&tmKV);
+      int stage = 0;
+      uint32_t phase = 0;
+      for (int u = blockIdx.x, it = 0; u < n_units; u += gridDim.x, ++it) {
+        const int qt = u % p.n_tiles, bh = u / p.n_tiles;
+        const int h = bh % p.H, b = bh / p.H;
+        auto load_q = [&]() {
+          if (it > 0) tc::mbar_wait_suspend(q_empty, (it - 1) & 1);
+          tc::mbar_expect_tx(q_full, 2 * ATT_TILE);
+          for (int g = 0; g < 2; ++g) att_load_tile(sQ + g * ATT_TILE, &tmQ, q_full, h * ATT_DH, b, qt * 128 + 64 * g);
+        };
+        const int claim_at = min(AF_STAGES - 1, nblk - 1);
+        if (nblk == 0) load_q();
+        for (int kb = 0; kb < nblk; ++kb) {
+          if (kb == claim_at) load_q();
+          tc::mbar_wait_suspend(&kv_empty[stage], phase ^ 1);
+          uint8_t* dst = sRing + stage * 2 * ATT_TILE;
+          tc::mbar_expect_tx(&kv_full[stage], 2 * ATT_TILE);
+          att_load_tile(dst, &tmKV, &kv_full[stage], E + h * ATT_DH, b, kb * ATT_TILE_ROWS);
+          att_load_tile(dst + ATT_TILE, &tmKV, &kv_full[stage], 2 * E + h * ATT_DH, b, kb * ATT_TILE_ROWS);
+          if (++stage == AF_STAGES) { stage = 0; phase ^= 1; }
+        }
+      }
+    }
+    return;
+  }
+
+  tc::setmaxnreg_inc<232>();
+  const int g = warp >> 2, wq = warp & 3;
+  const int tid = threadIdx.x & 127;
+  const uint32_t q_tile = tc::smem_u32(sQ + g * ATT_TILE);
+  uint8_t* stg = sStg + g * ATT_TILE;
+  const float dscale = p.drop_thr > 0 ? drop_scale(p.drop_thr) : 1.0f;
+  int stage = 0;
+  uint32_t phase = 0;
+  bool timed_out = false;
+  for (int u = blockIdx.x, it = 0; u < n_units && !timed_out; u += gridDim.x, ++it) {
+    const int qt = u % p.n_tiles, bh = u / p.n_tiles;
+    const int h = bh % p.H, b = bh / p.H;
+    const int t0 = qt * 128 + 64 * g;
+    const int i0 = t0 + 16 * wq + (lane >> 2);
+
+    float o[64], m[2], l[2];
+    uint32_t drow[2];
+#pragma unroll
+    for (int r = 0; r < 2; ++r) {
+      const int i = i0 + 8 * r;
+      const bool diag = i < p.T && i >= p.sep;
+      drow[r] = static_cast<uint32_t>(bh) * p.T + i;
+      const __nv_bfloat16* qrow = p.qkv + att_tok(diag ? i : 0, b, p.T, p.B, p.batch_major) * p.ld_qkv + h * ATT_DH;
+      float sd = 0.f;
+      if (diag) {
+#pragma unroll
+        for (int j = 0; j < 16; ++j) {
+          const float2 q = att_ld2(qrow, j, lane), k = att_ld2(qrow + E, j, lane);
+          sd = fmaf(q.x, k.x, fmaf(q.y, k.y, sd));
+        }
+      }
+      sd = quad_sum(sd) * p.scale_log2;
+      m[r] = diag ? sd : -INFINITY;
+      l[r] = diag && (lane & 3) == 0 ? 1.f : 0.f;
+      const bool keep = diag && (p.drop_thr == 0 || drop_keep(p.drop_seed, drow[r], i, p.drop_thr));
+#pragma unroll
+      for (int j = 0; j < 16; ++j) {
+        const float2 v = keep ? att_ld2(qrow + 2 * E, j, lane) : make_float2(0.f, 0.f);
+        o[4 * j + 2 * r] = v.x;
+        o[4 * j + 2 * r + 1] = v.y;
+      }
+    }
+    if (!tc::mbar_wait_bounded(q_full, it & 1)) { timed_out = true; break; }
+
+    float s[32];
+    uint32_t ap[16];
     float corr[2];
+    auto issue_s = [&](int st) {
+      const uint32_t k_s = tc::smem_u32(sRing + st * 2 * ATT_TILE);
+      const uint32_t q_s = att_opaque(q_tile);
+      tc::wgmma_fence();
+#pragma unroll
+      for (int kk = 0; kk < 8; ++kk) att_mma_n64(s, att_desc_k(q_s, kk), att_desc_k(k_s, kk), kk);
+      tc::wgmma_commit();
+    };
+    auto issue_pv = [&](int st) {
+      const uint32_t v_s = tc::smem_u32(sRing + st * 2 * ATT_TILE) + ATT_TILE;
+      tc::wgmma_fence();
+#pragma unroll
+      for (int kk = 0; kk < 4; ++kk) tc::wgmma_m64n128k16_rs(o, ap + 4 * kk, att_desc_mn(v_s, kk), 1);
+      tc::wgmma_commit();
+    };
+    auto softmax = [&](int kb) {
+      const int key0 = kb * ATT_TILE_ROWS + 2 * (lane & 3);
+      if (kb * ATT_TILE_ROWS + ATT_TILE_ROWS > p.sep) {
+#pragma unroll
+        for (int e = 0; e < 32; ++e)
+          if (key0 + 8 * (e >> 2) + (e & 1) >= p.sep) s[e] = -INFINITY;
+      }
+      float mx[2] = {-INFINITY, -INFINITY};
+#pragma unroll
+      for (int e = 0; e < 32; ++e) mx[(e >> 1) & 1] = fmaxf(mx[(e >> 1) & 1], s[e]);
+#pragma unroll
+      for (int r = 0; r < 2; ++r) {
+        const float mn = fmaxf(m[r], quad_max(mx[r]) * p.scale_log2);
+        corr[r] = fast_ex2(m[r] - mn);
+        m[r] = mn;
+        l[r] *= corr[r];
+      }
+#pragma unroll
+      for (int e = 0; e < 32; ++e) {
+        const int r = (e >> 1) & 1;
+        const float pr = fast_ex2(fmaf(s[e], p.scale_log2, -m[r]));
+        l[r] += pr;
+        s[e] = p.drop_thr > 0 && !drop_keep(p.drop_seed, drow[r], key0 + 8 * (e >> 2) + (e & 1), p.drop_thr) ? 0.f : pr;
+      }
+    };
+    auto rescale_pack = [&]() {
+#pragma unroll
+      for (int e = 0; e < 64; ++e) o[e] *= corr[(e >> 1) & 1];
+#pragma unroll
+      for (int e = 0; e < 16; ++e) ap[e] = tc::pack_bf16x2(s[2 * e], s[2 * e + 1]);
+    };
+    if (nblk > 0) {
+      if (!tc::mbar_wait_bounded(&kv_full[stage], phase)) { timed_out = true; break; }
+      issue_s(stage);
+      tc::wgmma_wait<0>();
+      tc::wgmma_fence_regs(s);
+      if (nblk == 1 && tid == 0) tc::mbar_arrive(q_empty);
+      softmax(0);
+      rescale_pack();
+      int cur = stage;
+      if (++stage == AF_STAGES) { stage = 0; phase ^= 1; }
+      for (int kb = 1; kb < nblk; ++kb) {
+        if (!timed_out && !tc::mbar_wait_bounded(&kv_full[stage], phase)) timed_out = true;
+        issue_s(stage);
+        issue_pv(cur);
+        tc::wgmma_wait<1>();
+        tc::wgmma_fence_regs(s);
+        if (kb == nblk - 1 && tid == 0) tc::mbar_arrive(q_empty);
+        softmax(kb);
+        tc::wgmma_wait<0>();
+        tc::wgmma_fence_regs(o);
+        if (tid == 0) tc::mbar_arrive(&kv_empty[cur]);
+        cur = stage;
+        if (++stage == AF_STAGES) { stage = 0; phase ^= 1; }
+        rescale_pack();
+      }
+      issue_pv(cur);
+      tc::wgmma_wait<0>();
+      tc::wgmma_fence_regs(o);
+      if (timed_out) break;
+      if (tid == 0) tc::mbar_arrive(&kv_empty[cur]);
+    } else if (tid == 0) {
+      tc::mbar_arrive(q_empty);
+    }
+
+    if (tid == 0) tc::bulk_wait_read<0>();
+    tc::named_bar_sync(1 + g, 128);
 #pragma unroll
     for (int r = 0; r < 2; ++r) {
-      const float mn = fmaxf(m[r], quad_max(mx[r]));
-      corr[r] = fast_ex2(m[r] - mn);
-      m[r] = mn;
-      l[r] *= corr[r];
-    }
-#pragma unroll
-    for (int j = 0; j < 8; ++j)
-#pragma unroll
-      for (int e = 0; e < 4; ++e) {
-        const float pr = fast_ex2(s[j][e] - m[e >> 1]);
-        l[e >> 1] += pr;
-        if (p.drop_thr > 0 && !drop_keep(p.drop_seed, drow0 + 8 * (e >> 1), key0 + 8 * j + (e & 1), p.drop_thr)) s[j][e] = 0.f;
-        else s[j][e] = pr;
-      }
-#pragma unroll
-    for (int j = 0; j < 16; ++j) {
-      o[j][0] *= corr[0]; o[j][1] *= corr[0];
-      o[j][2] *= corr[1]; o[j][3] *= corr[1];
-    }
-#pragma unroll
-    for (int kk = 0; kk < 4; ++kk) {
-      uint32_t a[4];
-      a[0] = tc::pack_bf16x2(s[2 * kk][0], s[2 * kk][1]);
-      a[1] = tc::pack_bf16x2(s[2 * kk][2], s[2 * kk][3]);
-      a[2] = tc::pack_bf16x2(s[2 * kk + 1][0], s[2 * kk + 1][1]);
-      a[3] = tc::pack_bf16x2(s[2 * kk + 1][2], s[2 * kk + 1][3]);
-#pragma unroll
-      for (int dp = 0; dp < 8; ++dp) {
-        uint32_t bb[4];
-        att_frag_bt(bb, v_s, kk * 16, dp * 16, lane);
-        tc::mma_bf16_16816(o[2 * dp], a, bb[0], bb[1]);
-        tc::mma_bf16_16816(o[2 * dp + 1], a, bb[2], bb[3]);
-      }
-    }
-    __syncthreads();
-  }
-
-  const float dscale = p.drop_thr > 0 ? drop_scale(p.drop_thr) : 1.0f;
-#pragma unroll
-  for (int r = 0; r < 2; ++r) {
-    const int i = i0 + r0 + (lane >> 2) + 8 * r;
-    float lr = quad_sum(l[r]);
-    const bool valid = i < p.T;
-    const bool diag = valid && i >= p.sep;
-    const __nv_bfloat16* qrow = p.qkv + att_tok(valid ? i : 0, b, p.T, p.B, p.batch_major) * p.ld_qkv + h * ATT_DH;
-    float sd = 0.f;
-    if (diag) {
+      const int i = i0 + 8 * r;
+      const float lr = quad_sum(l[r]);
+      const float inv = dscale / lr;
+      const int rr = 16 * wq + (lane >> 2) + 8 * r;
 #pragma unroll
       for (int j = 0; j < 16; ++j) {
-        const float2 q = att_ld2(qrow, j, lane), k = att_ld2(qrow + E, j, lane);
-        sd = fmaf(q.x, k.x, fmaf(q.y, k.y, sd));
-      }
-    }
-    sd = quad_sum(sd) * p.scale_log2;
-    if (diag) {
-      const float mn = fmaxf(m[r], sd);
-      const float c = fast_ex2(m[r] - mn);
-      const float pr = fast_ex2(sd - mn);
-      lr = lr * c + pr;
-      m[r] = mn;
-      const float pd = (p.drop_thr > 0 && !drop_keep(p.drop_seed, drow0 + 8 * r, i, p.drop_thr)) ? 0.f : pr;
-#pragma unroll
-      for (int j = 0; j < 16; ++j) {
-        const float2 v = att_ld2(qrow + 2 * E, j, lane);
-        o[j][2 * r] = fmaf(pd, v.x, o[j][2 * r] * c);
-        o[j][2 * r + 1] = fmaf(pd, v.y, o[j][2 * r + 1] * c);
-      }
-    }
-    if (valid) {
-      const float inv = dscale / lr;
-      __nv_bfloat16* orow = p.out + att_tok(i, b, p.T, p.B, p.batch_major) * p.ld_out + h * ATT_DH;
-#pragma unroll
-      for (int j = 0; j < 16; ++j) att_st2(orow, j, lane, o[j][2 * r] * inv, o[j][2 * r + 1] * inv);
-      if ((lane & 3) == 0) p.lse[static_cast<size_t>(bh) * p.T + i] = (m[r] + __log2f(lr)) * 0.69314718055994531f;
-    }
-  }
+        const uint32_t off = (j >> 3) * 8192 + rr * 128 + (((j & 7) ^ (rr & 7)) << 4) + (lane & 3) * 4;
+        *reinterpret_cast<uint32_t*>(stg + off) = tc::pack_bf16x2(o[4 * j + 2 * r] * inv, o[4 * j + 2 * r + 1] * inv);
+      }
+      if (i < p.T && (lane & 3) == 0) p.lse[static_cast<size_t>(bh) * p.T + i] = (m[r] + __log2f(lr)) * 0.69314718055994531f;
+    }
+    tc::fence_proxy_async_smem();
+    tc::named_bar_sync(1 + g, 128);
+    if (tid == 0 && t0 < p.T) {
+      tc::tma_store_3d(&tmO, stg, h * ATT_DH, b, t0);
+      tc::tma_store_3d(&tmO, stg + 8192, h * ATT_DH + 64, b, t0);
+      tc::bulk_commit();
+    }
+  }
+  if (tid == 0) tc::bulk_wait<0>();
+  if (timed_out) asm volatile("trap;");
 }
 
 }
@@ -177,18 +242,22 @@
   p.T = d->T; p.B = d->B; p.H = d->H; p.sep = d->sep;
   p.scale_log2 = d->scale * 1.4426950408889634f;
   p.qkv = reinterpret_cast<const __nv_bfloat16*>(d->qkv); p.ld_qkv = d->ld_qkv;
-  p.out = reinterpret_cast<__nv_bfloat16*>(d->out); p.ld_out = d->ld_out;
   p.lse = d->lse;
-  p.n_qtiles = (d->T + ATT_BM - 1) / ATT_BM;
+  p.n_tiles = (d->T + 127) / 128;
   p.batch_major = d->batch_major;
   p.drop_seed = d->drop_seed; p.drop_thr = d->drop_thr;
-  const long long grid = static_cast<long long>(p.n_qtiles) * d->B * d->H;
-  PFN_CHECK_ARG(grid < (1LL << 31), "attention_fwd_tc: too many tiles");
+  const int E = d->H * ATT_DH;
+  CUtensorMap tmQ, tmKV, tmO;
+  if (int rc = att_qkv_maps(d, &tmQ, &tmKV)) return rc;
+  if (int rc = att_tensor_map(&tmO, d->out, E, d->ld_out, d->T, d->B, d->T, d->batch_major)) return rc;
+  const long long units = static_cast<long long>(p.n_tiles) * d->B * d->H;
+  PFN_CHECK_ARG(units < (1LL << 31), "attention_fwd_tc: too many tiles");
   static bool attr_set[64] = {};
   if (first_use_on_device(attr_set)) {
-    PFN_CUDA_OK(cudaFuncSetAttribute(attn_fwd_tc_kernel, cudaFuncAttributeMaxDynamicSharedMemorySize, ATT_FWD_SMEM));
-  }
-  attn_fwd_tc_kernel<<<static_cast<unsigned>(grid), 128, ATT_FWD_SMEM, reinterpret_cast<cudaStream_t>(stream)>>>(p);
+    PFN_CUDA_OK(cudaFuncSetAttribute(attn_fwd_kernel, cudaFuncAttributeMaxDynamicSharedMemorySize, AF_SMEM));
+  }
+  const int grid = units < num_sms() ? static_cast<int>(units) : num_sms();
+  attn_fwd_kernel<<<static_cast<unsigned>(grid), AF_THREADS, AF_SMEM, reinterpret_cast<cudaStream_t>(stream)>>>(tmQ, tmKV, tmO, p);
   PFN_LAUNCH_OK();
   return 0;
 }
diff --git a/transformerscandobayesianinference_b200/csrc/tc_common.cuh b/transformerscandobayesianinference_b200/csrc/tc_common.cuh
--- a/transformerscandobayesianinference_b200/csrc/tc_common.cuh
+++ b/transformerscandobayesianinference_b200/csrc/tc_common.cuh
@@ -83,6 +83,11 @@
 __device__ __forceinline__ void tma_store_2d(const CUtensorMap* m, const void* smem_src, int c0, int c1) {
   asm volatile("cp.async.bulk.tensor.2d.global.shared::cta.tile.bulk_group [%0, {%2, %3}], [%1];"
                ::"l"(reinterpret_cast<uint64_t>(m)), "r"(smem_u32(smem_src)), "r"(c0), "r"(c1)
+               : "memory");
+}
+__device__ __forceinline__ void tma_store_3d(const CUtensorMap* m, const void* smem_src, int c0, int c1, int c2) {
+  asm volatile("cp.async.bulk.tensor.3d.global.shared::cta.tile.bulk_group [%0, {%2, %3, %4}], [%1];"
+               ::"l"(reinterpret_cast<uint64_t>(m)), "r"(smem_u32(smem_src)), "r"(c0), "r"(c1), "r"(c2)
                : "memory");
 }
 __device__ __forceinline__ void tma_reduce_add_2d(const CUtensorMap* m, const void* smem_src, int c0, int c1) {
@@ -196,32 +201,6 @@
       : "r"(a[0]), "r"(a[1]), "r"(a[2]), "r"(a[3]), "l"(b_desc), "r"(accumulate));
 }
 
-__device__ __forceinline__ void mma_bf16_16816(float (&c)[4], const uint32_t (&a)[4], uint32_t b0, uint32_t b1) {
-  asm volatile(
-      "mma.sync.aligned.m16n8k16.row.col.f32.bf16.bf16.f32 {%0, %1, %2, %3}, {%4, %5, %6, %7}, {%8, %9}, "
-      "{%0, %1, %2, %3};"
-      : "+f"(c[0]), "+f"(c[1]), "+f"(c[2]), "+f"(c[3])
-      : "r"(a[0]), "r"(a[1]), "r"(a[2]), "r"(a[3]), "r"(b0), "r"(b1));
-}
-__device__ __forceinline__ void ldmatrix_x4(uint32_t (&r)[4], uint32_t addr) {
-  asm volatile("ldmatrix.sync.aligned.m8n8.x4.shared.b16 {%0, %1, %2, %3}, [%4];"
-               : "=r"(r[0]), "=r"(r[1]), "=r"(r[2]), "=r"(r[3])
-               : "r"(addr));
-}
-__device__ __forceinline__ void ldmatrix_x4_trans(uint32_t (&r)[4], uint32_t addr) {
-  asm volatile("ldmatrix.sync.aligned.m8n8.x4.trans.shared.b16 {%0, %1, %2, %3}, [%4];"
-               : "=r"(r[0]), "=r"(r[1]), "=r"(r[2]), "=r"(r[3])
-               : "r"(addr));
-}
-__device__ __forceinline__ void cp_async16(uint32_t dst, const void* src, uint32_t src_bytes) {
-  asm volatile("cp.async.cg.shared.global [%0], [%1], 16, %2;" ::"r"(dst), "l"(src), "r"(src_bytes) : "memory");
-}
-__device__ __forceinline__ void cp_async_commit() { asm volatile("cp.async.commit_group;" ::: "memory"); }
-template <int N>
-__device__ __forceinline__ void cp_async_wait() {
-  asm volatile("cp.async.wait_group %0;" ::"n"(N) : "memory");
-}
-
 }
 
 int make_tensor_map(CUtensorMap* out, const void* base, bool f32, int rank, const uint64_t* dims,
```

New measurement: 2385, median of 6. 1.04x the previous value.
